# SixLabors/ZlibStream

Measured on AMD Instinct MI355X. Metric: deflate MB/s (input) at level 6, 64 MiB buffers, higher is better.
Workload: dtype u8; 1 GPU; english64: 1 x 67108864-byte pseudo-random-English (Zipf words of alice29.txt) buffer per GPU, level 6, zlib framing, inputs resident in HBM; level=6, buffer_bytes=67108864, buffers_per_gpu=1, compressed_bytes=27425826, parallelism=independent buffers, 1 GPU(s), no collective in the data path

## Files before the change

### zlibstream_amd/csrc/zs_core.h

```cpp
#pragma once
#include <stdint.h>
#include <vector>

#if defined(__HIPCC__)
#include <hip/hip_runtime.h>
#define ZS_HD __host__ __device__ __forceinline__
#define ZS_HD_NOINLINE __host__ __device__
#else
#define ZS_HD inline
#define ZS_HD_NOINLINE
#endif

namespace zs {

constexpr int kMinMatch = 3;
constexpr int kMaxMatch = 258;
constexpr int kMinLookahead = kMaxMatch + kMinMatch + 1;
constexpr int kWSize = 32768;
constexpr int kWMask = kWSize - 1;
constexpr int kWindowSize = 2 * kWSize;
constexpr int kMaxDist = kWSize - kMinLookahead;
constexpr int kSlideAt = kWindowSize - kMinLookahead;
constexpr int kHashBits = 15;
constexpr int kHashSize = 1 << kHashBits;
// ... 417 lines not shown
        uint32_t cK = acc.mK(p), cK4 = acc.mK4(p);
        if (p == 0) cK = cK4 = kNoMatch;
        Step st = lazy_step(kind, p, pend, cK, cK4, lv);
        if (st.emit) {
            uint32_t sym = st.emit == 1 ? (uint32_t)acc.byte(p - 1) : (((uint32_t)st.dist << 16) | (uint32_t)(st.len - 3));
            sink(ns, sym, st.emit == 1 ? p : p - 1 + st.len, p);
            ns++;
        }
        if (st.kind == kXK) pend = cK;
        else if (st.kind == kXK4) pend = cK4;
        kind = st.kind;
        p = st.pos;
    }
    exit_slot = kind == kR ? (int)(p - cx.ce) : 256 + kind;
    nsyms = ns;
}

constexpr int kJumpRounds = 12;
ZS_HD uint32_t node_pack(int succ, int cnt) { return (uint32_t)succ | ((uint32_t)cnt << 14); }
ZS_HD int node_succ(uint32_t v) { return (int)(v & 0x3FFF); }
ZS_HD int node_cnt(uint32_t v) { return (int)(v >> 14); }
ZS_HD uint32_t node_jump(uint32_t v, uint32_t w) { return node_pack(node_succ(w), node_cnt(v) + node_cnt(w)); }

constexpr int kNodeExit3 = 3 * kChunk;
static_assert(kNodeExit3 + 512 <= (1 << 14), "node ids and exit codes share 14 bits");
ZS_HD int kind_row(int kind) { return kind == kR ? 0 : kind == kXK4 ? 2 : 1; }
ZS_HD int node_of3(int kind, int64_t p, int64_t cs, int64_t ce) {
    return p < ce ? kind_row(kind) * kChunk + (int)(p - cs) : kNodeExit3 + (kind == kR ? (int)(p - ce) : 256 + kind);
}
template <class Acc>
ZS_HD uint32_t node_step3(const Acc &acc, int row, int64_t p, int64_t cs, int64_t ce, const LevelCfg &lv) {
    const uint32_t before = acc.mK(p - 1);
    const int kind = row == 0 ? kR : row == 2 ? kXK4 : (before != kNoMatch ? kXK : kL);
    const uint32_t pend = kind == kXK ? before : kind == kXK4 ? acc.mK4(p - 1) : kNoMatch;
    uint32_t cK = acc.mK(p), cK4 = acc.mK4(p);
    if (p == 0) cK = cK4 = kNoMatch;
    const Step st = lazy_step(kind, p, pend, cK, cK4, lv);
    return node_pack(node_of3(st.kind, st.pos, cs, ce), st.emit ? 1 : 0);
}
template <class Acc>
ZS_HD void node_step3_all(const Acc &acc, int64_t p, int64_t cs, int64_t ce, const LevelCfg &lv, uint32_t &r0, uint32_t &r1, uint32_t &r2) {
    const uint32_t before = acc.mK(p - 1), before4 = acc.mK4(p - 1);
    uint32_t cK = acc.mK(p), cK4 = acc.mK4(p);
    if (p == 0) cK = cK4 = kNoMatch;
    const Step s0 = lazy_step(kR, p, kNoMatch, cK, cK4, lv);
    const Step s1 = lazy_step(before != kNoMatch ? kXK : kL, p, before, cK, cK4, lv);
    const Step s2 = lazy_step(kXK4, p, before4, cK, cK4, lv);
    r0 = node_pack(node_of3(s0.kind, s0.pos, cs, ce), s0.emit ? 1 : 0);
    r1 = node_pack(node_of3(s1.kind, s1.pos, cs, ce), s1.emit ? 1 : 0);
    r2 = node_pack(node_of3(s2.kind, s2.pos, cs, ce), s2.emit ? 1 : 0);
}
template <class Acc, class Tbl>
ZS_HD uint32_t chunk_exit_by_table3(const Acc &acc, const Tbl &tbl, const ChunkCtx &cx, int slot, const LevelCfg &lv, int strategy) {
    const int64_t ce = cx.ce;
    int kind, ns;
    int64_t p;
    uint32_t flags;
    NullSink nsink;
    NullEv nev;
    chunk_special_prefix(acc, nsink, cx, slot, lv, strategy, kind, p, ns, flags, nev);
    while (p < ce && (kind == kL || kind == kXK) && ((kind == kXK) != (acc.mK(p - 1) != kNoMatch))) {
        const uint32_t pend = kind == kXK ? acc.mK(p - 1) : kNoMatch;
        uint32_t cK = acc.mK(p), cK4 = acc.mK4(p);
        if (p == 0) cK = cK4 = kNoMatch;
        const Step st = lazy_step(kind, p, pend, cK, cK4, lv);
        if (st.emit) ns++;
        kind = st.kind;
        p = st.pos;
    }
    int node = node_of3(kind, p, cx.cs, ce);
    while (node < kNodeExit3) {
        const uint32_t v = tbl[node];
        ns += node_cnt(v);
        node = node_succ(v);
    }
    return (uint32_t)(node - kNodeExit3) | flags | ((uint32_t)ns << 16);
}

constexpr int kSpecSlabPad = 32;
constexpr int kSpecMaxLenBits = 11;
ZS_HD constexpr int spec_slab_stride(int len_bits) { return (1 << len_bits) + kSpecSlabPad; }
ZS_HD int sym_len(uint32_t sym) { return (sym >> 16) ? (int)(sym & 0xFFFFu) + kMinMatch : 1; }
ZS_HD int spec_cut_index(uint32_t base, int count) {
    const uint32_t i = (base / (uint32_t)kBlockSyms + 1u) * (uint32_t)kBlockSyms - 1u - base;
    return i < (uint32_t)count ? (int)i : -1;
}
ZS_HD int64_t spec_first_start(int64_t cs, int slot) { return slot <= 256 ? cs + slot : cs - 1; }
ZS_HD int64_t spec_sym_end(int64_t start, uint32_t sym) { return start + sym_len(sym); }
ZS_HD int64_t spec_sym_top(int64_t start, bool odd) { return start + (odd ? 2 : 1); }
struct SpecSlabSink {
    uint32_t *out;
    int odd;
    ZS_HD void operator()(int i, uint32_t sym, int64_t end, int64_t top) {
        out[i] = sym;
        if (top != spec_sym_top(end - sym_len(sym), false)) odd = i;
    }
};

ZS_HD bool slot_valid(const ChunkCtx &cx, int slot, int64_t body_end) {
    if (slot <= 256) return cx.cs + slot <= body_end + 257;
    return cx.cs > 0;
}


ZS_HD int extra_lbits(int code) { return code < 8 ? 0 : (code == 28 ? 0 : (code - 4) >> 2); }
ZS_HD int extra_dbits(int code) { return code < 4 ? 0 : (code - 2) >> 1; }
ZS_HD int extra_blbits(int code) { return code == 16 ? 2 : code == 17 ? 3 : code == 18 ? 7 : 0; }
ZS_HD int base_length(int code) {
    if (code < 8) return code;
    if (code == 28) return 0;
    int e = (code - 4) >> 2;
    return ((4 + (code & 3)) << e);
}
ZS_HD int length_code(int lc) {
    if (lc < 8) return lc;
    if (lc == 255) return 28;
    int e = 31 - __builtin_clz((unsigned)lc) - 2;
    return 4 * e + 4 + ((lc >> e) & 3);
}
ZS_HD int base_dist(int code) {
    if (code < 4) return code;
    int e = (code - 2) >> 1;
    return (2 + (code & 1)) << e;
}
ZS_HD int dist_code(int d) {
    if (d < 4) return d;
    int e = 31 - __builtin_clz((unsigned)d) - 1;
    return 2 * e + 2 + ((d >> e) & 1);
}
ZS_HD int bl_order(int i) {
    const uint8_t t[19] = {16, 17, 18, 0, 8, 7, 9, 6, 10, 5, 11, 4, 12, 3, 13, 2, 14, 1, 15};
    return t[i];
}
ZS_HD unsigned bit_reverse(unsigned code, int len) {
    unsigned r = 0;
    for (int i = 0; i < len; i++) {
        r = (r << 1) | (code & 1u);
        code >>= 1;
    }
    return r;
}
ZS_HD int static_llen(int n) { return n <= 143 ? 8 : n <= 255 ? 9 : n <= 279 ? 7 : 8; }
ZS_HD unsigned static_lcode(int n) {
    unsigned c = n <= 143 ? 0x30 + n : n <= 255 ? 0x190 + (n - 144) : n <= 279 ? (unsigned)(n - 256) : 0xC0 + (n - 280);
    return bit_reverse(c, static_llen(n));
}

struct CtData {
    uint16_t fc;
    uint16_t dl;
};

struct TreeWork {
    CtData ltree[kHeapSize];
    CtData dtree[2 * kDCodes + 1];
    CtData bltree[2 * kBlCodes + 1];
    uint16_t heap[kHeapSize];
    uint8_t depth[kHeapSize];
    uint16_t bl_count[kMaxBits + 1];
    int heap_len, heap_max;
    int opt_len, static_len;
    int l_max_code, d_max_code, max_blindex;
};

struct TreeDesc {
    int which;
    int elems, max_length, extra_base;
};
ZS_HD int desc_extra(const TreeDesc &d, int n) {
    if (n < d.extra_base) return 0;
    n -= d.extra_base;
    return d.which == 0 ? extra_lbits(n) : d.which == 1 ? extra_dbits(n) : extra_blbits(n);
}
ZS_HD int desc_static_len(const TreeDesc &d, int n) { return d.which == 0 ? static_llen(n) : 5; }

ZS_HD_NOINLINE inline void gen_bitlen(TreeWork &w, CtData *tree, int max_code, const TreeDesc &d) {
    int h, n, m, bits, overflow = 0;
    for (bits = 0; bits <= kMaxBits; bits++) w.bl_count[bits] = 0;
    tree[w.heap[w.heap_max]].dl = 0;
    for (h = w.heap_max + 1; h < kHeapSize; h++) {
        n = w.heap[h];
        bits = tree[tree[n].dl].dl + 1;
        if (bits > d.max_length) {
            bits = d.max_length;
            overflow++;
        }
        tree[n].dl = (uint16_t)bits;
        if (n > max_code) continue;
        w.bl_count[bits]++;
        int xbits = desc_extra(d, n);
        int f = tree[n].fc;
        w.opt_len += f * (bits + xbits);
        if (d.which != 2) w.static_len += f * (desc_static_len(d, n) + xbits);
    }
    if (overflow == 0) return;
    do {
        bits = d.max_length - 1;
        while (w.bl_count[bits] == 0) bits--;
        w.bl_count[bits]--;
        w.bl_count[bits + 1] += 2;
        w.bl_count[d.max_length]--;
        overflow -= 2;
    } while (overflow > 0);
    for (bits = d.max_length; bits != 0; bits--) {
        n = w.bl_count[bits];
        while (n != 0) {
            m = w.heap[--h];
            if (m > max_code) continue;
            if (tree[m].dl != (unsigned)bits) {
                w.opt_len += bits * (int)tree[m].fc;
                w.opt_len -= (int)tree[m].dl * (int)tree[m].fc;
                tree[m].dl = (uint16_t)bits;
            }
            n--;
        }
    }
}

ZS_HD_NOINLINE inline void gen_codes(CtData *tree, int max_code, const uint16_t *bl_count) {
    uint16_t next_code[kMaxBits + 1];
    unsigned code = 0;
    next_code[0] = 0;
    for (int bits = 1; bits <= kMaxBits; bits++) {
        code = (code + bl_count[bits - 1]) << 1;
        next_code[bits] = (uint16_t)code;
    }
    for (int n = 0; n <= max_code; n++) {
        int len = tree[n].dl;
        if (len == 0) continue;
        tree[n].fc = (uint16_t)bit_reverse(next_code[len]++, len);
    }
}

ZS_HD uint32_t hk_pack(uint32_t freq, uint32_t depth, uint32_t node) { return (freq << 16) | (depth << 10) | node; }
ZS_HD void pqdownheap_packed(uint32_t *hk, int len, int k) {
    const uint32_t v = hk[k];
    int j = k << 1;
    while (j <= len) {
        uint32_t c = hk[j];
        const uint32_t c1 = hk[j + 1];
        const int gj = j << 1;
        const uint32_t g0 = hk[gj], g1 = hk[gj + 1], g2 = hk[gj + 2], g3 = hk[gj + 3];
        if (j < len && (c1 >> 10) <= (c >> 10)) c = c1, j++;
        if ((v >> 10) <= (c >> 10)) break;
        hk[k] = c;
        k = j;
        j <<= 1;
        if (j > len) break;
        uint32_t e = (k & 1) ? g2 : g0;
        const uint32_t e1 = (k & 1) ? g3 : g1;
        if (j < len && (e1 >> 10) <= (e >> 10)) e = e1, j++;
        if ((v >> 10) <= (e >> 10)) break;
        hk[k] = e;
        k = j;
        j <<= 1;
    }
    hk[k] = v;
}
ZS_HD_NOINLINE inline int build_tree(TreeWork &w, uint32_t *hk, CtData *tree, const TreeDesc &d) {
    int max_code = -1, node, len = 0;
    w.heap_max = kHeapSize;
    for (int n = 0; n < d.elems; n++) {
        if (tree[n].fc != 0) {
            hk[++len] = hk_pack(tree[n].fc, 0, (uint32_t)(max_code = n));
        } else {
            tree[n].dl = 0;
        }
    }
    while (len < 2) {
        node = max_code < 2 ? ++max_code : 0;
        hk[++len] = hk_pack(1, 0, (uint32_t)node);
        tree[node].fc = 1;
        w.opt_len--;
        if (d.which != 2) w.static_len -= desc_static_len(d, node);
    }
    for (int n = len / 2; n >= 1; n--) pqdownheap_packed(hk, len, n);
    node = d.elems;
    do {
        const uint32_t n = hk[1];
        hk[1] = hk[len--];
        pqdownheap_packed(hk, len, 1);
        const uint32_t m = hk[1];
        w.heap[--w.heap_max] = (uint16_t)(n & 1023u);
        w.heap[--w.heap_max] = (uint16_t)(m & 1023u);
        const uint32_t f = (n >> 16) + (m >> 16), dn = (n >> 10) & 63u, dm = (m >> 10) & 63u;
        tree[node].fc = (uint16_t)f;
        tree[n & 1023u].dl = tree[m & 1023u].dl = (uint16_t)node;
        hk[1] = hk_pack(f, (dn >= dm ? dn : dm) + 1, (uint32_t)node);
        node++;
        pqdownheap_packed(hk, len, 1);
    } while (len >= 2);
    w.heap[--w.heap_max] = (uint16_t)(hk[1] & 1023u);
    w.heap_len = len;
    gen_bitlen(w, tree, max_code, d);
    gen_codes(tree, max_code, w.bl_count);
    return max_code;
}

ZS_HD_NOINLINE inline void scan_tree(TreeWork &w, CtData *tree, int max_code) {
    int prevlen = -1, curlen, nextlen = tree[0].dl, count = 0, max_count = 7, min_count = 4;
    if (nextlen == 0) max_count = 138, min_count = 3;
    tree[max_code + 1].dl = 0xFFFF;
    for (int n = 0; n <= max_code; n++) {
        curlen = nextlen;
        nextlen = tree[n + 1].dl;
        if (++count < max_count && curlen == nextlen) continue;
        if (count < min_count) {
            w.bltree[curlen].fc += (uint16_t)count;
        } else if (curlen != 0) {
            if (curlen != prevlen) w.bltree[curlen].fc++;
            w.bltree[16].fc++;
        } else if (count <= 10) {
            w.bltree[17].fc++;
        } else {
            w.bltree[18].fc++;
        }
        count = 0;
        prevlen = curlen;
        if (nextlen == 0) max_count = 138, min_count = 3;
        else if (curlen == nextlen) max_count = 6, min_count = 3;
        else max_count = 7, min_count = 4;
    }
}

ZS_HD_NOINLINE inline int build_block_trees(TreeWork &w, uint32_t *hk, int stored_len, bool can_store, int strategy) {
    w.opt_len = w.static_len = 0;
    for (int i = 0; i < kBlCodes; i++) w.bltree[i].fc = 0;
    const TreeDesc ld = {0, kLCodes, kMaxBits, kLiterals + 1};
    const TreeDesc dd = {1, kDCodes, kMaxBits, 0};
    const TreeDesc bd = {2, kBlCodes, kMaxBlBits, 0};
    w.l_max_code = build_tree(w, hk, w.ltree, ld);
    w.d_max_code = build_tree(w, hk, w.dtree, dd);
    scan_tree(w, w.ltree, w.l_max_code);
    scan_tree(w, w.dtree, w.d_max_code);
    build_tree(w, hk, w.bltree, bd);
    int mb;
    for (mb = kBlCodes - 1; mb >= 3; mb--)
        if (w.bltree[bl_order(mb)].dl != 0) break;
    w.max_blindex = mb;
    w.opt_len += 3 * (mb + 1) + 5 + 5 + 4;
    int opt_lenb = (w.opt_len + 3 + 7) >> 3;
    int static_lenb = (w.static_len + 3 + 7) >> 3;
    if (static_lenb <= opt_lenb) opt_lenb = static_lenb;
    if (stored_len + 4 <= opt_lenb && can_store) return 0;
    if (strategy == kFixed || static_lenb == opt_lenb) return 1;
    return 2;
}

template <class LT, class DT>
ZS_HD int encode_symbol(const LT &lt, const DT &dt, int dist, int lc, uint64_t &bits) {
    if (dist == 0) {
        bits = lt[lc].fc;
        return lt[lc].dl;
    }
    int code = length_code(lc);
    uint64_t b = lt[code + kLiterals + 1].fc;
    int n = lt[code + kLiterals + 1].dl;
    int extra = extra_lbits(code);
    if (extra) {
        b |= (uint64_t)(lc - base_length(code)) << n;
        n += extra;
    }
    int d = dist - 1;
    code = dist_code(d);
    b |= (uint64_t)dt[code].fc << n;
    n += dt[code].dl;
    extra = extra_dbits(code);
    if (extra) {
        b |= (uint64_t)(d - base_dist(code)) << n;
        n += extra;
    }
    bits = b;
    return n;
}

struct StaticLTree {
    struct E {
        uint16_t fc, dl;
    };
    ZS_HD E operator[](int n) const { return {(uint16_t)static_lcode(n), (uint16_t)static_llen(n)}; }
};
struct StaticDTree {
    struct E {
        uint16_t fc, dl;
    };
    ZS_HD E operator[](int n) const { return {(uint16_t)bit_reverse((unsigned)n, 5), 5}; }
};


template <class Put>
ZS_HD_NOINLINE inline void emit_tree_rle(const CtData *tree, int max_code, const CtData *bl, Put &put) {
    int prevlen = -1, curlen, nextlen = tree[0].dl, count = 0, max_count = 7, min_count = 4;
    if (nextlen == 0) max_count = 138, min_count = 3;
    for (int n = 0; n <= max_code; n++) {
        curlen = nextlen;
        nextlen = tree[n + 1].dl;
        if (++count < max_count && curlen == nextlen) continue;
        if (count < min_count) {
            do put(bl[curlen].fc, bl[curlen].dl);
            while (--count != 0);
        } else if (curlen != 0) {
            if (curlen != prevlen) {
                put(bl[curlen].fc, bl[curlen].dl);
                count--;
            }
            put(bl[16].fc, bl[16].dl);
            put((unsigned)(count - 3), 2);
        } else if (count <= 10) {
            put(bl[17].fc, bl[17].dl);
            put((unsigned)(count - 3), 3);
        } else {
            put(bl[18].fc, bl[18].dl);
            put((unsigned)(count - 11), 7);
        }
        count = 0;
        prevlen = curlen;
        if (nextlen == 0) max_count = 138, min_count = 3;
        else if (curlen == nextlen) max_count = 6, min_count = 3;
        else max_count = 7, min_count = 4;
    }
}

template <class Put>
ZS_HD_NOINLINE inline void emit_dyn_header(const TreeWork &w, Put &put) {
    int lcodes = w.l_max_code + 1, dcodes = w.d_max_code + 1, blcodes = w.max_blindex + 1;
    put((unsigned)(lcodes - 257), 5);
    put((unsigned)(dcodes - 1), 5);
    put((unsigned)(blcodes - 4), 4);
    for (int rank = 0; rank < blcodes; rank++) put(w.bltree[bl_order(rank)].dl, 3);
    emit_tree_rle(w.ltree, lcodes - 1, w.bltree, put);
    emit_tree_rle(w.dtree, dcodes - 1, w.bltree, put);
}

ZS_HD unsigned zlib_header(int level) {
    unsigned header = (8u + (7u << 4)) << 8;
    unsigned lf = (((unsigned)(level - 1)) & 0xFF) >> 1;
    if (lf > 3) lf = 3;
    header |= lf << 6;
    header += 31 - (header % 31);
    return header;
}

constexpr uint32_t kAdlerBase = 65521;
ZS_HD uint32_t adler_combine(uint32_t a1, uint32_t a2, uint64_t len2) {
    uint32_t rem = (uint32_t)(len2 % kAdlerBase);
    uint32_t s1a = a1 & 0xFFFF, s2a = a1 >> 16, s1b = a2 & 0xFFFF, s2b = a2 >> 16;
    uint64_t s1 = (uint64_t)s1a + s1b + kAdlerBase - 1;
    uint64_t s2 = (uint64_t)s2a + s2b + (uint64_t)rem * ((s1a + kAdlerBase - 1) % kAdlerBase);
    return (uint32_t)(((s2 % kAdlerBase) << 16) | (s1 % kAdlerBase));
}

struct FlushAcct {
// ... 167 lines not shown
```

### zlibstream_amd/csrc/zs_engine.hip

```cpp
#include <hip/hip_runtime.h>

#include <algorithm>
#include <cstdio>
#include <cstdlib>
#include <cstring>
#include <string>
#include <thread>
#include <vector>

#define ZS_BUILDING_LIBRARY
#include "../../include/zsgpu.h"
#include "zs_kernels.hip"
#include "zs_inflate_par.hip"
#include "zs_inflate_tok.hip"
#include "zs_png.hip"
#include "zs_crc32.hip"

using namespace zs;

namespace {

struct DevBuf {
    void *p = nullptr;
    size_t cap = 0;
};

enum Stage {
    kStClear, kStAdler, kStLinks, kStMatch, kStChunkMap, kStSegMap, kStResolve, kStExpand, kStEmitSyms, kStTail, kStTrees,
    kStOffsets, kStEmitBits, kStSpecWalk, kStSpecVerify, kStCrc32, kStSpecCompact, kStPngExpand, kStCount
};
const char *const kStageNames[kStCount] = {"clear", "adler", "links", "match", "chunkmap", "segmap", "resolve", "expand",
                                           "emit_syms", "tail", "trees", "offsets", "emit_bits", "spec_walk", "spec_verify", "crc32_frame",
                                           "spec_compact", "png_expand"};

}

struct zs_ctx {
    int device = 0;
    hipStream_t stream = nullptr;
    hipStream_t aux = nullptr;
    hipEvent_t ev_fork = nullptr, ev_join = nullptr, ev_pre0 = nullptr, ev_pre = nullptr;
    hipEvent_t ev_spec[4] = {};
    std::string err;
    bool profiling = false;
    int fast_fallbacks = 0;
    int round_runs = 0;
    int cut_rounds = 0;
    int lit_fallbacks = 0;
    int spec_streams = 0, spec_fallbacks = 0, spec_wrong_chunks = 0;
    int spec_periodic = 0;
    int64_t dbg_blk_off = 0, dbg_chunk_off = 0, dbg_nchunks = 0, dbg_spec_n = 0, dbg_n_spec = 0;
    int64_t lit_engine_bytes = 0;
    std::vector<int64_t> inf_used;
    int64_t *inf_probe = nullptr;
    int inf_lane_streams = 0;
    int inf_wave_streams = 0;
    int64_t png_segments = 0;
    int fast_rounds = 0;
    bool no_rounds_once = false;
    int last_op = 0;
    hipEvent_t ev[kStCount + 1] = {};
    double stage_ms[kStCount] = {};
    uint32_t *crc_tab = nullptr;
    DevBuf sd, st, work, wpre, geo, link, mm, maps, chunk_far, segmap, supmap, seg_entry, seg_symbase, seg_stale, entry, symbase, stale, syms, blk_end, blk_top, blocks, trees, info, pieces, scratch,
        stage_in, stage_out, wr, inf_desc, inf_state, par_ps, par_st, par_work, par_cbits, par_ccnt, par_surv, par_scnt, par_cands, par_tabs, par_toktabs, par_toks, par_ctoks, par_tokstat, par_tails, par_retry, par_fxtab, par_blocks, par_cells,
        par_windows, par_fail, run_syms, run_bits, run_scratch, run_outs, run_fail, adl_tr, adl_res, plan_blk, ins_bits, mm_bak, cut_pos, cut_bkt, win_groups, win_sg, win_maps, win_entries, persist_bak, resume_flag, rle_tiles, own_in, fr_chunks, fr_meta, fr_planes, fr_prov, fr_base, fr_counters, spec_rec, spec_flags, spec_syms, png_img, png_seg, png_ctr, png_fimg, png_scratch, png_a7img, png_inflated, png_passes, crc_desc, crc_res, png_zs, png_gather, png_ximg, png_raw;
    uint32_t *crc32_tab = nullptr;
    hipEvent_t ev_crc[2] = {};
    hipEvent_t ev_expand[2] = {};
    bool resume_poisoned = false;
    void *pinned = nullptr;
    size_t pinned_cap = 0;
    void *pin_io = nullptr;
    size_t pin_io_cap = 0;
    bool pin_io_busy = false;
    void *pin_out = nullptr;
    size_t pin_out_cap = 0;
    bool pin_out_busy = false;
};

namespace {

bool fail(zs_ctx *c, const char *what, hipError_t e) {
    c->err = std::string(what) + ": " + hipGetErrorString(e);
    return false;
}
#define ZS_HIP(c, call)                                  \
    do {                                                 \
        hipError_t e_ = (call);                          \
        if (e_ != hipSuccess) return fail(c, #call, e_); \
    } while (0)

bool ensure(zs_ctx *c, DevBuf &b, size_t bytes) {
    if (bytes <= b.cap) return true;
    if (b.p) (void)hipFree(b.p);
    b.p = nullptr;
    b.cap = 0;
    size_t want = bytes + bytes / 8 + 4096;
    if (hipMalloc(&b.p, want) != hipSuccess) {
        (void)hipGetLastError();
        b.p = nullptr;
        want = bytes + 4096;
        if (hipMalloc(&b.p, want) != hipSuccess) {
            (void)hipGetLastError();
            b.p = nullptr;
            char msg[160];
            snprintf(msg, sizeof msg, "workspace: %zu bytes do not fit the device's free memory (the pipeline needs ~17 bytes per input byte: split the batch)", bytes);
            c->err = msg;
            return false;
        }
    }
    b.cap = want;
    return true;
}
bool ensure_pinned(zs_ctx *c, size_t bytes) {
    if (bytes <= c->pinned_cap) return true;
    if (c->pinned) (void)hipHostFree(c->pinned);
    c->pinned = nullptr;
    c->pinned_cap = 0;
    ZS_HIP(c, hipHostMalloc(&c->pinned, bytes + 4096, hipHostMallocDefault));
    c->pinned_cap = bytes + 4096;
    return true;
}

struct WorkList {
    std::vector<int32_t> pre;
    void add(int stream, int64_t count) {
        while ((int)pre.size() <= stream) pre.push_back(pre.empty() ? 0 : pre.back());
        pre.push_back(pre.back() + (int32_t)count);
    }
    void finish(int n) {
        if (pre.empty()) pre.push_back(0);
        while ((int)pre.size() <= n) pre.push_back(pre.back());
    }
    size_t size() const { return pre.empty() ? 0 : (size_t)pre.back(); }
    bool empty() const { return size() == 0; }
};
constexpr int kWorkLists = 9;
struct Plan {
    std::vector<StreamDesc> sd;
    WorkList w_clear, w_adler, w_links, w_match, w_chunks, w_segs, w_sups, w_blocks, w_runs;
    int64_t n_pos = 0, n_syms = 0;
    int64_t n_chunks = 0, n_segs = 0, n_sups = 0, n_blocks = 0, n_pieces = 0, n_runs = 0;
    int64_t n_spec = 0;
    int max_spec_n = 0, n_spec_streams = 0;
    bool any_fv = false, any_rle = false;
    bool any_dual = false;
    int64_t n_rle_tiles = 0;
    int64_t lit_bytes = 0;
    std::vector<FsChunk> fr_chunks;
    size_t fr_prov = 0;
    int fr_max_n = 0;
    int64_t n_cuts = 0;
    std::vector<int32_t> seg_c0, seg_after, seg_base, seg_S, seg_cl, cstart, head;
    std::vector<uint32_t> cl;
    std::vector<BlockRec> plan_blk;
    std::vector<int32_t> plan_wr_blk;
};

template <class T>
T *dev(DevBuf &b) {
    return (T *)b.p;
}

struct WriteSpec {
    std::vector<int64_t> ends;
    std::vector<uint8_t> flush;
    int chunk = 512;
    bool raw = false;
    bool flushing() const {
        for (uint8_t f : flush)
            if (f) return true;
        return false;
    }
};

struct RunOpts {
    bool final_run = true, cont = false;
    int64_t hist = 0;
    LitPersist *persist = nullptr;
    int64_t abs_off = 0;
    uint32_t adler_stream = 1, carry_byte = 0;
    int64_t end_bits = 0;
    int64_t stop_abs = -1;
    bool resume = false, mid_write = false, at_read = false;
    int64_t p0 = 0, E0 = 0, base0 = 0, start_block = 0;
    int slot = 0;
    uint32_t start_syms = 0;
};

bool run_pipeline(zs_ctx *c, int n, const void *const *in, const int64_t *in_len, void *const *out, const int64_t *out_cap,
                  int64_t *out_len, int *status, int level, int strategy, int hash_variant, hipStream_t stream,
                  const WriteSpec *const *writes = nullptr, int force_seq = 0, RunOpts *ro = nullptr, bool rounds = false,
                  const std::vector<uint8_t> *force_lit = nullptr) {
    if (level == -1) level = 6;
    LevelCfg lv = level_cfg(level);
    static const bool host_times = getenv("ZS_HOST_TIMES") != nullptr;
    const auto ht0 = std::chrono::steady_clock::now();
    auto ht_us = [&]() { return std::chrono::duration<double, std::micro>(std::chrono::steady_clock::now() - ht0).count(); };
    double ht_plan = 0, ht_launched = 0;
    for (int i = 0; i < n; i++) {
        out_len[i] = 0;
        if (status) status[i] = ZS_STREAM_ERROR;
    }
    bool any_writes = false;
    for (int i = 0; i < n && writes; i++) any_writes = any_writes || writes[i] != nullptr;
    if (any_writes && n > 1)
        for (int i = 0; i < n; i++)
            if (ro || (writes[i] && writes[i]->flushing())) {
                c->err = "flush modes and incremental runs take one stream a call";
                return false;
            }
    std::vector<WriteSpec> rle_one;
    std::vector<const WriteSpec *> rle_writes;
    if (any_writes && strategy == kRle && level >= 1 && !ro && !getenv("ZS_NO_RLE_MULTI")) {
        rle_one.resize((size_t)n);
        rle_writes.assign(writes, writes + n);
// ... 141 lines not shown
                    pl.seg_S.push_back(0), pl.seg_cl.push_back((int32_t)pl.cl.size());
                    s.nsegs++;
                }
            pl.seg_cl.push_back((int32_t)pl.cl.size());
            pl.cstart.push_back(0);
        }
        s.seg_c0 = s.seg_after = s.seg_base = s.seg_S = s.seg_cl = nullptr, s.cl = nullptr, s.cstart = nullptr, s.head = nullptr;
        pl.n_segs += s.nsegs;
        s.sup_off = (int32_t)pl.n_sups;
        pl.n_sups += (s.nsegs + kSupSegs - 1) / kSupSegs;
        s.spec = 0, s.spec_n = 0, s.spec_off = (int32_t)pl.n_spec;
        bool spec_geo = s.body_end >= 0 && geo.body_end == len - kMinLookahead;
        if (spec_geo) {
            const int64_t want = 1 + (len > kWindowSize ? (len - kWindowSize - 1) / kWSize + 1 : 0);
            spec_geo = (int64_t)geo.nsegs() == want && geo.seg_cl.size() == (size_t)want + 1 && geo.seg_cl[0] == 0 && geo.seg_cl[1] == 0;
            for (int64_t k = 1; k < want && spec_geo; k++)
                spec_geo = geo.seg_cl[(size_t)k + 1] - geo.seg_cl[(size_t)k] == 1 &&
                           geo.cl[(size_t)geo.seg_cl[(size_t)k]] == ((uint32_t)(kWindowSize + kWSize * (k - 1)) | kClWindowBit);
        }
        if (spec_on && lv.func == 2 && (strategy == kDefault || strategy == kFiltered) && !wr && !ro && !lit_forced && spec_geo && len >= spec_min &&
            n <= 65535) {
            s.spec = 1, s.spec_n = (int32_t)((((int64_t)s.body_end + kMinLookahead - 1) >> spec_bits) + 1);
            pl.n_spec += s.spec_n, pl.n_spec_streams++;
            pl.max_spec_n = std::max(pl.max_spec_n, (int)s.spec_n);
        }
        s.run_chunk = run_chunk;
        s.fast_runs = fast_par ? (force_seq == 2 ? 1 : (int32_t)((len + run_chunk - 1) / run_chunk)) : 0;
        s.run_slots = fast_par ? (force_seq == 2 ? (int32_t)((len + 4096) / kFastChunk + 1) : s.fast_runs) : 0;
        s.run_off = (int32_t)pl.n_runs;
        pl.n_runs += s.run_slots;
        pl.w_runs.add(i, s.fast_runs);
        s.blk_off = (int32_t)pl.n_blocks;
        s.max_blocks = (int32_t)(level == 0 ? len / 8191 + len / 32506 + 4 : len / kBlockSyms + 2);
        if (flushing) s.max_blocks += (int32_t)wr->ends.size() + 1;
        s.plan_blk = nullptr, s.plan_nblk = 0;
        s.final_run = final_run ? 1 : 0, s.cont = cont ? 1 : 0, s.persist = ro ? ro->persist : nullptr;
        s.abs_off = (ro && !resume) ? ro->abs_off : 0, s.adler_stream = ro ? ro->adler_stream : 1, s.carry_byte = ro ? ro->carry_byte : 0;
        if (level == 0 && strategy != kRle && !ro) {
            const size_t first = pl.plan_blk.size();
            const std::vector<int64_t> no_ends;
            const std::vector<uint8_t> no_flush;
            if (flushing) pl.plan_wr_blk.assign(wr->ends.size(), 0);
            plan_stored_blocks(len, (multi || flushing) ? wr->ends : no_ends, flushing ? wr->flush : no_flush,
                               [&](int64_t start, int32_t blen, int can_store, int eof) {
                                   pl.plan_blk.push_back(BlockRec{start, 0, blen, 0, can_store, eof});
                               },
                               [&](int w, int nb) {
                                   if (flushing) pl.plan_wr_blk[(size_t)w] = nb;
                               });
            s.plan_nblk = (int32_t)(pl.plan_blk.size() - first);
            s.plan_blk = (const BlockRec *)(uintptr_t)first;
            s.max_blocks = s.plan_nblk + 1;
        }
        pl.n_blocks += s.max_blocks;
        s.adler_off = (int32_t)pl.n_pieces;
        s.n_adler = ro ? 0 : (int32_t)((len + kAdlerPiece - 1) / kAdlerPiece);
        pl.n_pieces += s.n_adler;
        pl.w_clear.add(i, (s.out_cap + 65535) / 65536);
        pl.w_adler.add(i, s.n_adler);
        if (s.body_end >= 0 || s.fast_runs > 0 || s.fv_end >= 0)
            pl.w_links.add(i, len - 5 > 0 ? (len - 5 + link_span - 1) / link_span : 0);
        if (s.body_end >= 0) {
            pl.w_match.add(i, (int64_t)s.body_end / kMatchTile + 1);
            pl.w_chunks.add(i, s.nchunks);
            pl.w_segs.add(i, s.nsegs);
            if (s.nsegs > kSupSegs) pl.w_sups.add(i, (s.nsegs + kSupSegs - 1) / kSupSegs);
        }
        pl.w_blocks.add(i, s.max_blocks);
        if (s.body_end < 0 && s.fv_end < 0 && s.rle_end < 0 && s.fast_runs == 0 && s.plan_nblk == 0 && !(level == 0 && strategy != kRle && !ro)) {
            const int64_t from = resume ? ro->p0 : ro ? ro->hist : 0;
            pl.lit_bytes += std::max<int64_t>(0, len - from - (kMinLookahead - 1));
        }
    }
    {
        int64_t need = 0;
        for (int i = 0; i < n; i++) need += (pl.sd[(size_t)i].spec_n + 63) / 64;
        if (pl.n_spec && (int64_t)((pl.max_spec_n + 63) / 64) * n > 4 * need + 4096) {
            for (int i = 0; i < n; i++) pl.sd[(size_t)i].spec = 0, pl.sd[(size_t)i].spec_n = 0, pl.sd[(size_t)i].spec_off = 0;
            pl.n_spec = 0, pl.max_spec_n = 0, pl.n_spec_streams = 0;
        }
    }
    if (allow_dual && dual_broken) {
        allow_dual = false, dual_broken = false;
        goto plan_again;
    }
    pl.any_dual = allow_dual;
    c->lit_engine_bytes += pl.lit_bytes;
    auto plan_rerun = [&]() { c->lit_engine_bytes -= pl.lit_bytes; };
    c->fast_rounds = 0;
    const bool no_rounds_this_call = c->no_rounds_once;
    c->no_rounds_once = false;
    if (pl.any_fv && !getenv("ZS_FAST_NO_ROUNDS") && !no_rounds_this_call && !(ro && ro->resume && getenv("ZS_NO_RESUME_ROUNDS"))) {
        int64_t pos_fv = 0, max_fv = 0;
        for (int i = 0; i < n; i++)
            if (pl.sd[(size_t)i].fv_end >= 0) {
                pos_fv += pl.sd[(size_t)i].fv_end + 1 - pl.sd[(size_t)i].start_pos;
                max_fv = std::max<int64_t>(max_fv, pl.sd[(size_t)i].fv_end + 1 - pl.sd[(size_t)i].start_pos);
            }
        const double t_stream = (double)max_fv / (level >= 3 ? 20e6 : level == 2 ? 35e6 : 46e6);
        const double t_rounds = std::min(0.016, (double)max_fv / 60e6) + (double)pos_fv / 3.5e9;
        if (getenv("ZS_FR_RATIO") ? (double)pos_fv <= atof(getenv("ZS_FR_RATIO")) * (double)max_fv : t_rounds < t_stream) {
            int64_t target = getenv("ZS_FR_CHUNK") ? atoll(getenv("ZS_FR_CHUNK")) : pos_fv / 250;
            target = target < 2048 ? 2048 : target > kFsChunkMax ? kFsChunkMax : target;
            bool too_short = false;
            for (;;) {
                pl.fr_chunks.clear();
                pl.fr_max_n = 0;
                too_short = false;
                for (int i = 0; i < n; i++) {
                    StreamDesc &s = pl.sd[(size_t)i];
                    if (s.fv_end < 0) continue;
                    s.fr_first = (int32_t)pl.fr_chunks.size();
                    {
                        const int32_t *after = pl.seg_after.data() + s.seg_off;
                        const bool res = s.resume != 0;
                        const int64_t shortest = fs_build_chunks(i, (int64_t)s.fv_end, s.nsegs - 1, [&](int k) { return (int64_t)after[k - 1] - (kMinLookahead - 1); }, (int)target, pl.fr_chunks,
                                                                 res ? 2 : 1, res ? s.start_pos : 0);
                        if (shortest < kFsMinSpan) too_short = true;
                    }
                    s.fr_n = (int32_t)pl.fr_chunks.size() - s.fr_first;
                    pl.fr_max_n = s.fr_n > pl.fr_max_n ? s.fr_n : pl.fr_max_n;
                }
                if (pl.fr_chunks.size() <= 256 || target >= kFsChunkMax || getenv("ZS_FR_CHUNK")) break;
                target += 128;
            }
            if (too_short) {
                pl.fr_chunks.clear();
                pl.fr_max_n = 0;
                for (int i = 0; i < n; i++) pl.sd[(size_t)i].fr_first = pl.sd[(size_t)i].fr_n = 0;
            }
            for (FsChunk &ck : pl.fr_chunks) {
                ck.prov_off = (uint32_t)pl.fr_prov;
                pl.fr_prov += (size_t)(ck.b_hi - ck.b_lo) + kMaxMatch + 64;
            }
            if (pl.fr_prov > 0xFFFF0000u) {
                pl.fr_chunks.clear();
                pl.fr_max_n = 0, pl.fr_prov = 0;
                for (int i = 0; i < n; i++) pl.sd[(size_t)i].fr_first = pl.sd[(size_t)i].fr_n = 0;
            }
        }
    }
    WorkList *const lists[kWorkLists] = {&pl.w_clear, &pl.w_adler, &pl.w_links, &pl.w_match, &pl.w_chunks, &pl.w_segs, &pl.w_sups, &pl.w_blocks, &pl.w_runs};
    for (WorkList *l : lists) l->finish(n);
    size_t n_work = pl.w_clear.size() + pl.w_adler.size() + pl.w_links.size() + pl.w_match.size() + pl.w_chunks.size() +
                    pl.w_segs.size() + pl.w_sups.size() + pl.w_blocks.size() + pl.w_runs.size();
    if (!ensure(c, c->sd, sizeof(StreamDesc) * (size_t)n) || !ensure(c, c->st, sizeof(StreamState) * (size_t)n) ||
        !ensure(c, c->work, sizeof(uint2) * (n_work + 1)) || !ensure(c, c->link, 2 * (size_t)pl.n_pos + 64) ||
        !ensure(c, c->mm, 8 * (size_t)pl.n_pos + 256) ||
        !ensure(c, c->maps, 4 * (size_t)(pl.n_chunks + 1) * kSlots) || !ensure(c, c->segmap, 8 * (size_t)(pl.n_segs + 1) * kSlots) ||
        !ensure(c, c->supmap, 8 * (size_t)(pl.n_sups + 1) * kSlots) || !ensure(c, c->chunk_far, 2 * (size_t)pl.n_chunks + 64) ||
        !ensure(c, c->seg_entry, 2 * (size_t)(pl.n_segs + 2)) || !ensure(c, c->seg_symbase, 4 * (size_t)(pl.n_segs + 2)) ||
        !ensure(c, c->seg_stale, (size_t)pl.n_segs + 64) || !ensure(c, c->entry, 2 * (size_t)(pl.n_chunks + 2)) ||
        !ensure(c, c->symbase, 4 * (size_t)(pl.n_chunks + 2)) || !ensure(c, c->stale, (size_t)pl.n_chunks + 64) ||
        !ensure(c, c->syms, 4 * (size_t)pl.n_syms + 64) || !ensure(c, c->blk_end, 4 * (size_t)pl.n_blocks + 64) ||
        !ensure(c, c->blk_top, 4 * (size_t)pl.n_blocks + 64) || !ensure(c, c->blocks, sizeof(BlockRec) * (size_t)pl.n_blocks) ||
        !ensure(c, c->trees, sizeof(TreeWork) * (size_t)pl.n_blocks) || !ensure(c, c->info, sizeof(BlockInfo) * (size_t)pl.n_blocks) ||
        !ensure(c, c->pieces, 4 * (size_t)pl.n_pieces + 64) || !ensure(c, c->scratch, (size_t)kScratchBytes * (size_t)n) ||
        !ensure(c, c->cut_pos, 8 * (size_t)pl.n_cuts + 64) || !ensure(c, c->cut_bkt, 8 * (size_t)pl.n_cuts + 64) ||
        (pl.n_spec && (!ensure(c, c->spec_rec, 8 * (size_t)pl.n_spec + 64) || !ensure(c, c->spec_flags, 4 * (size_t)n + 64) ||
                       !ensure(c, c->spec_syms, 4 * (size_t)pl.n_spec * (size_t)spec_slab_stride(spec_bits) + 64))))
        return false;
    const size_t o_segcl = 16 * (size_t)pl.n_segs, o_cstart = o_segcl + 4 * ((size_t)pl.n_segs + (size_t)n),
                 o_head = o_cstart + 4 * ((size_t)pl.n_chunks + (size_t)n), o_cl = o_head + 4 * (size_t)pl.n_chunks;
    const size_t geo_bytes = o_cl + 4 * pl.cl.size();
    if (!ensure(c, c->geo, geo_bytes + 64)) return false;
    for (int i = 0; i < n; i++) {
        StreamDesc &s = pl.sd[(size_t)i];
        const int32_t *g = (const int32_t *)c->geo.p;
        const uint8_t *gb = (const uint8_t *)c->geo.p;
        s.seg_c0 = g + s.seg_off, s.seg_after = g + pl.n_segs + s.seg_off, s.seg_base = g + 2 * pl.n_segs + s.seg_off;
        s.seg_S = g + 3 * pl.n_segs + s.seg_off;
        s.seg_cl = (const int32_t *)(gb + o_segcl) + s.seg_off + i;
        s.cstart = (const int32_t *)(gb + o_cstart) + s.chunk_off + i;
        s.head = (const int32_t *)(gb + o_head) + s.chunk_off;
        s.cl = (const uint32_t *)(gb + o_cl);
    }
    if (pl.any_fv) {
        if (!ensure(c, c->ins_bits, (size_t)pl.n_pos / 8 + kFvBitSlack)) return false;
        for (int i = 0; i < n; i++)
            if (pl.sd[(size_t)i].fv_end >= 0) pl.sd[(size_t)i].ins_bits = dev<uint32_t>(c->ins_bits) + pl.sd[(size_t)i].pos_off / 32;
    }
    if (!pl.plan_blk.empty()) {
        if (!ensure(c, c->plan_blk, sizeof(BlockRec) * pl.plan_blk.size())) return false;
        for (int i = 0; i < n; i++)
            if (pl.sd[(size_t)i].plan_nblk) pl.sd[(size_t)i].plan_blk = dev<BlockRec>(c->plan_blk) + (uintptr_t)pl.sd[(size_t)i].plan_blk;
    }
    if (pl.n_runs &&
        (!ensure(c, c->run_syms, 4 * (size_t)pl.n_runs * kFastRunSyms) || !ensure(c, c->run_bits, 4 * (size_t)pl.n_runs * kFastRunBitWords) ||
         !ensure(c, c->run_scratch, (size_t)pl.n_runs * kFastRunScratch) || !ensure(c, c->run_outs, sizeof(FastRunOut) * (size_t)pl.n_runs) ||
         !ensure(c, c->run_fail, 4 * (size_t)n + 64)))
        return false;
    if (any_writes) {
        std::vector<size_t> nws((size_t)n, 0), offs;
        for (int i = 0; i < n; i++) {
            const WriteSpec *wr = writes[i];
            if (wr && (wr->ends.size() > 1 || wr->flushing() || ro)) nws[(size_t)i] = wr->ends.size();
        }
        const size_t wr_bytes = layout_write_blocks(nws, offs);
        if (!ensure(c, c->wr, wr_bytes + 64)) return false;
        std::vector<uint8_t> hw(rounds ? 0 : wr_bytes + 64, 0);
        for (int i = 0; i < n; i++) {
            const WriteSpec *wr = writes[i];
            const size_t nw = nws[(size_t)i];
            if (!wr || !(wr->ends.size() > 1 || wr->flushing() || ro)) continue;
            uint8_t *blk = (uint8_t *)c->wr.p + offs[(size_t)i];
            pl.sd[(size_t)i].wr_end = (const int64_t *)blk;
            if (wr->flushing() || ro) {
                pl.sd[(size_t)i].wr_blk = (int32_t *)(blk + 8 * nw);
                pl.sd[(size_t)i].wr_flush = blk + 12 * nw;
            }
            if (rounds || !nw) continue;
            memcpy(hw.data() + offs[(size_t)i], wr->ends.data(), sizeof(int64_t) * nw);
            if (wr->flushing() || ro) memcpy(hw.data() + offs[(size_t)i] + 12 * nw, wr->flush.data(), nw);
            if (!pl.plan_wr_blk.empty()) memcpy(hw.data() + offs[(size_t)i] + 8 * nw, pl.plan_wr_blk.data(), 4 * nw);
        }
        if (!rounds && wr_bytes) {
            ZS_HIP(c, hipMemcpyAsync(c->wr.p, hw.data(), hw.size(), hipMemcpyHostToDevice, stream));
            ZS_HIP(c, hipStreamSynchronize(stream));
        }
    }
    if (!rounds && !pl.plan_blk.empty()) {
        ZS_HIP(c, hipMemcpyAsync(c->plan_blk.p, pl.plan_blk.data(), sizeof(BlockRec) * pl.plan_blk.size(), hipMemcpyHostToDevice, stream));
        ZS_HIP(c, hipStreamSynchronize(stream));
    }
    const size_t pre_bytes = 4 * (size_t)kWorkLists * (size_t)(n + 1);
    size_t up_bytes = sizeof(StreamDesc) * (size_t)n + pre_bytes + geo_bytes + 16;
    if (!ensure_pinned(c, std::max(up_bytes, sizeof(StreamState) * (size_t)n)) || !ensure(c, c->wpre, pre_bytes + 64)) return false;
    uint8_t *hp = (uint8_t *)c->pinned;
    memcpy(hp, pl.sd.data(), sizeof(StreamDesc) * (size_t)n);
    int32_t *hpre = (int32_t *)(hp + sizeof(StreamDesc) * (size_t)n);
    size_t o_clear = 0, o_adler, o_links, o_match, o_chunks, o_segs, o_sups, o_blocks, o_runs;
    WorkOffsets wo;
    {
        size_t *const offs[kWorkLists] = {&o_clear, &o_adler, &o_links, &o_match, &o_chunks, &o_segs, &o_sups, &o_blocks, &o_runs};
        size_t at = 0;
        for (int l = 0; l < kWorkLists; l++) {
            *offs[l] = at;
            wo.off[l] = (uint32_t)at;
            memcpy(hpre + (size_t)l * (size_t)(n + 1), lists[l]->pre.data(), 4 * (size_t)(n + 1));
            at += lists[l]->size();
        }
        wo.off[kWorkLists] = (uint32_t)at;
    }
    if (geo_bytes) {
        uint8_t *hg = hp + sizeof(StreamDesc) * (size_t)n + pre_bytes;
        if (pl.n_segs) {
            memcpy(hg, pl.seg_c0.data(), 4 * (size_t)pl.n_segs);
            memcpy(hg + 4 * (size_t)pl.n_segs, pl.seg_after.data(), 4 * (size_t)pl.n_segs);
            memcpy(hg + 8 * (size_t)pl.n_segs, pl.seg_base.data(), 4 * (size_t)pl.n_segs);
            memcpy(hg + 12 * (size_t)pl.n_segs, pl.seg_S.data(), 4 * (size_t)pl.n_segs);
        }
        memcpy(hg + o_segcl, pl.seg_cl.data(), 4 * pl.seg_cl.size());
        memcpy(hg + o_cstart, pl.cstart.data(), 4 * pl.cstart.size());
        if (pl.n_chunks) memcpy(hg + o_head, pl.head.data(), 4 * (size_t)pl.n_chunks);
        if (!pl.cl.empty()) memcpy(hg + o_cl, pl.cl.data(), 4 * pl.cl.size());
        if (!rounds) ZS_HIP(c, hipMemcpyAsync(c->geo.p, hg, geo_bytes, hipMemcpyHostToDevice, stream));
    }
    if (!rounds) ZS_HIP(c, hipMemcpyAsync(c->sd.p, hp, sizeof(StreamDesc) * (size_t)n, hipMemcpyHostToDevice, stream));
    if (n_work && !rounds) {
        ZS_HIP(c, hipMemcpyAsync(c->wpre.p, hpre, pre_bytes, hipMemcpyHostToDevice, stream));
        hipLaunchKernelGGL(zs_worklist_kernel, dim3((unsigned)((n_work + 255) / 256)), dim3(256), 0, stream, dev<int32_t>(c->wpre), n, wo,
                           dev<uint2>(c->work));
    }
    if (!rounds) {
        ZeroRegions z;
        auto reg = [&](int r, DevBuf &b, size_t bytes) {
            z.p[r] = b.p;
            z.n16[r] = (uint32_t)(((bytes + 15) / 16 < b.cap / 16) ? (bytes + 15) / 16 : b.cap / 16);
        };
        reg(0, c->stale, (size_t)pl.n_chunks + 64);
        reg(1, c->seg_stale, (size_t)pl.n_segs + 64);
        reg(2, c->st, sizeof(StreamState) * (size_t)n);
        if (pl.any_fv) reg(3, c->ins_bits, (size_t)pl.n_pos / 8 + kFvBitSlack);
        else z.p[3] = nullptr, z.n16[3] = 0;
        uint32_t most = 0;
        for (int r = 0; r < 4; r++) most = z.n16[r] > most ? z.n16[r] : most;
        unsigned blocks = (most + 255) / 256;
        if (blocks > 2048) blocks = 2048;
        if (blocks < 1) blocks = 1;
        hipLaunchKernelGGL(zs_zero_kernel, dim3(blocks), dim3(256), 0, stream, z);
        if (ro && ro->resume && pl.sd[0].fv_end >= 0) {
            const int64_t lo = std::max<int64_t>(0, ro->p0 - kWSize - 64) / 32, hi = ro->p0 / 32;
            if (hi > lo) ZS_HIP(c, hipMemsetAsync(pl.sd[0].ins_bits + lo, 0xFF, (size_t)(hi - lo) * 4, stream));
            ZS_HIP(c, hipMemsetD32Async((hipDeviceptr_t)(pl.sd[0].ins_bits + hi), (int)((1u << (ro->p0 & 31)) - 1u), 1, stream));
        }
    }

    const StreamDesc *d_sd = dev<StreamDesc>(c->sd);
    StreamState *d_st = dev<StreamState>(c->st);
    const uint2 *d_work = dev<uint2>(c->work);
    const bool prof = c->profiling;
    const int k5_ahead = getenv("ZS_K5_AHEAD") ? atoi(getenv("ZS_K5_AHEAD")) : 1;
    c->dbg_blk_off = pl.sd[0].blk_off, c->dbg_chunk_off = pl.sd[0].chunk_off, c->dbg_nchunks = pl.sd[0].nchunks;
    c->dbg_spec_n = pl.sd[0].spec_n, c->dbg_n_spec = pl.n_spec;
    const K5Spec k5s{dev<uint32_t>(c->spec_rec), dev<uint32_t>(c->spec_rec) + pl.n_spec, spec_bits, spec_warm, spec_corrupt,
                     dev<uint32_t>(c->spec_syms), spec_slab_stride(spec_bits)};
    int spec_ok_streams = 0;
    bool need_maps = true, spec_ran = false;
    if (!rounds) c->spec_streams = c->spec_fallbacks = c->spec_wrong_chunks = c->spec_periodic = 0;
    auto mark = [&](int i) {
        if (prof) (void)hipEventRecord(c->ev[i], stream);
    };
    ht_plan = ht_us();
    ZS_HIP(c, hipEventRecord(c->ev_pre0, stream));
    auto side_work = [&]() -> bool {
        ZS_HIP(c, hipStreamWaitEvent(c->aux, c->ev_pre0, 0));
        if (!pl.w_clear.empty())
            hipLaunchKernelGGL(zs_clear_kernel, dim3((unsigned)pl.w_clear.size()), dim3(256), 0, c->aux, d_sd, d_work + o_clear);
        if (!pl.w_adler.empty())
// ... 210 lines not shown
                    char b[64];
                    snprintf(b, sizeof b, " %u/%d(%.2f)", changed, fr.range, r <= g_n ? 0.0 : std::chrono::duration<double, std::milli>(t_now - t_last).count());
                    t_last = t_now;
                    trace += b;
                }
                if (!env_fixed) {
                    static const double env_wake = getenv("ZS_FR_WAKE") ? atof(getenv("ZS_FR_WAKE")) : 4.0;
                    const size_t awake = std::min<size_t>(nch, (size_t)(env_wake * (double)changed));
                    const int tail = env_tail;
                    fr.range = std::min<int>(range_max, std::max<int>(tail, (int)((awake + 255) / 256)));
                }
            }
            c->fast_rounds = r;
            if (env_dbg) fprintf(stderr, "zs: DeflateFast over %zu chunks of %d streams, up to %d to a workgroup: %d rounds (changed/range:%s)\n", nch, n, range_max, r, trace.c_str());
            if (changed) {
                ZS_HIP(c, hipStreamSynchronize(c->aux));
                c->no_rounds_once = true;
                return plan_rerun(), run_pipeline(c, n, in, in_len, out, out_cap, out_len, status, level, strategy, hash_variant, stream, writes, force_seq, ro, false, force_lit);
            }
            const FsMeta *mf = dev<FsMeta>(c->fr_meta) + (size_t)((r - 1) & 1) * nch;
            hipLaunchKernelGGL(zs_fast_commit_scan_kernel, dim3((unsigned)n), dim3(1024), 0, stream, d_sd, d_st, mf, dev<int32_t>(c->fr_base));
            hipLaunchKernelGGL(zs_fast_commit_kernel, dim3((unsigned)nch), dim3(256), 0, stream, d_sd, fr, mf, dev<int32_t>(c->fr_base), dev<uint16_t>(c->link),
                               dev<uint32_t>(c->syms), dev<int32_t>(c->blk_end), dev<int32_t>(c->blk_top));
        } else {
            hipLaunchKernelGGL((zs_fast_sweep_kernel<1024, kFsTile1, false>), dim3((unsigned)n), dim3(1024), fs_lds, stream, d_sd, d_st, dev<uint16_t>(c->link),
                               dev<uint32_t>(c->syms), dev<int32_t>(c->blk_end), dev<int32_t>(c->blk_top), lv, strategy, FsRounds());
        }
    }
    if (pl.any_rle) {
        const size_t nt = (size_t)pl.n_rle_tiles;
        if (!ensure(c, c->rle_tiles, 4 * (4 * nt + (size_t)n) + 256)) return false;
        int32_t *rb = dev<int32_t>(c->rle_tiles);
        RleTiles rt{rb, rb + nt, rb + 2 * nt, rb + 3 * nt, rb + 4 * nt};
        int max_tiles = 0;
        for (int i = 0; i < n; i++)
            if (pl.sd[(size_t)i].rle_end >= 0) max_tiles = std::max(max_tiles, (pl.sd[(size_t)i].rle_end + kMaxMatch + 1 + 4095) / 4096);
        auto tiles = [&](auto &&launch) {
            for (int s0 = 0; s0 < n; s0 += 65535) launch(dim3((unsigned)((max_tiles + 3) / 4), (unsigned)std::min(n - s0, 65535)), s0);
        };
        tiles([&](dim3 tg, int s0) { hipLaunchKernelGGL(zs_rle_starts_kernel, tg, dim3(256), 0, stream, d_sd, rt, s0); });
        hipLaunchKernelGGL(zs_rle_scan_kernel, dim3((unsigned)n), dim3(1024), 0, stream, d_sd, rt);
        tiles([&](dim3 tg, int s0) {
            hipLaunchKernelGGL(zs_rle_pass_kernel<0>, tg, dim3(256), 0, stream, d_sd, rt, dev<uint32_t>(c->syms), dev<int32_t>(c->blk_end), dev<int32_t>(c->blk_top), s0);
        });
        hipLaunchKernelGGL(zs_rle_sums_kernel, dim3((unsigned)n), dim3(1024), 0, stream, d_sd, d_st, rt);
        tiles([&](dim3 tg, int s0) {
            hipLaunchKernelGGL(zs_rle_pass_kernel<1>, tg, dim3(256), 0, stream, d_sd, rt, dev<uint32_t>(c->syms), dev<int32_t>(c->blk_end), dev<int32_t>(c->blk_top), s0);
        });
    }
    const bool tail_late = ro && (!ro->final_run || ro->resume);
    const bool tail_serial = !tail_late && n >= 64 && (pl.n_pos / n >= (96 << 10) || getenv("ZS_TAIL_SERIAL")) && !getenv("ZS_TAIL_FORK");
    if (!tail_late && !tail_serial) {
        ZS_HIP(c, hipEventRecord(c->ev_fork, stream));
        ZS_HIP(c, hipStreamWaitEvent(c->aux, c->ev_fork, 0));
        hipLaunchKernelGGL(zs_tail_kernel, dim3((unsigned)n), dim3(1024), kTailLds, c->aux, d_sd, d_st, dev<uint16_t>(c->link),
                           dev<uint32_t>(c->syms), dev<int32_t>(c->blk_end), dev<int32_t>(c->blk_top), dev<BlockRec>(c->blocks),
                           dev<uint8_t>(c->scratch), c->crc_tab, lv, strategy, hash_variant, level);
        ZS_HIP(c, hipEventRecord(c->ev_join, c->aux));
    }
    if (!pl.w_segs.empty() && need_maps)
        hipLaunchKernelGGL(zs_expand_kernel, dim3((unsigned)((pl.w_segs.size() + 63) / 64)), dim3(64), 0, stream, d_sd, d_st,
                           d_work + o_segs, (int)pl.w_segs.size(), dev<uint2>(c->mm), dev<uint16_t>(c->link),
                           dev<uint32_t>(c->maps), dev<uint16_t>(c->seg_entry), dev<uint32_t>(c->seg_symbase),
                           dev<uint8_t>(c->stale), dev<uint16_t>(c->entry), dev<uint32_t>(c->symbase), c->crc_tab, lv, strategy,
                           hash_variant);
    mark(8);
    if (!pl.w_chunks.empty() && need_maps)
        hipLaunchKernelGGL((zs_emit_syms_lane_kernel<4, 0>), dim3((unsigned)((pl.w_chunks.size() + 63) / 64)), dim3(kK5Threads), 0, stream, d_sd, d_st,
                           d_work + o_chunks, (int)pl.w_chunks.size(), dev<uint2>(c->mm), dev<uint16_t>(c->link), dev<uint16_t>(c->entry),
                           dev<uint32_t>(c->symbase), dev<uint32_t>(c->syms), dev<int32_t>(c->blk_end), dev<int32_t>(c->blk_top),
                           c->crc_tab, lv, strategy, hash_variant, k5_ahead, k5s);
    if (spec_ok_streams) {
        if (prof) (void)hipEventRecord(c->ev_spec[2], stream);
        hipLaunchKernelGGL(zs_spec_compact_kernel, dim3((unsigned)((pl.max_spec_n + 3) / 4), (unsigned)n), dim3(256), 0, stream, d_sd, d_st, k5s,
                           dev<uint32_t>(c->syms), dev<int32_t>(c->blk_end), dev<int32_t>(c->blk_top));
        if (prof) (void)hipEventRecord(c->ev_spec[3], stream);
    }
    mark(9);
    if (tail_serial)
        hipLaunchKernelGGL(zs_tail_kernel, dim3((unsigned)n), dim3(1024), kTailLds, stream, d_sd, d_st, dev<uint16_t>(c->link),
                           dev<uint32_t>(c->syms), dev<int32_t>(c->blk_end), dev<int32_t>(c->blk_top), dev<BlockRec>(c->blocks),
                           dev<uint8_t>(c->scratch), c->crc_tab, lv, strategy, hash_variant, level);
    else if (!tail_late) ZS_HIP(c, hipStreamWaitEvent(stream, c->ev_join, 0));
    hipLaunchKernelGGL(zs_body_blocks_kernel, dim3((unsigned)n), dim3(256), 0, stream, d_sd, d_st, dev<int32_t>(c->blk_end),
                       dev<int32_t>(c->blk_top), dev<BlockRec>(c->blocks), dev<uint32_t>(c->syms));
    if (tail_late)
        hipLaunchKernelGGL(zs_tail_kernel, dim3((unsigned)n), dim3(1024), kTailLds, stream, d_sd, d_st, dev<uint16_t>(c->link),
                           dev<uint32_t>(c->syms), dev<int32_t>(c->blk_end), dev<int32_t>(c->blk_top), dev<BlockRec>(c->blocks),
                           dev<uint8_t>(c->scratch), c->crc_tab, lv, strategy, hash_variant, level);
    if (pl.n_runs) {
        if (!getenv("ZS_FAST_NO_PROBE") && force_seq == 0 && !pl.any_dual) {
            hipLaunchKernelGGL(zs_fast_probe_kernel, dim3((unsigned)n), dim3(256), 0, stream, d_sd, dev<uint16_t>(c->link), dev<int32_t>(c->run_fail));
            std::vector<int32_t> np((size_t)n, 0);
            ZS_HIP(c, hipMemcpyAsync(np.data(), c->run_fail.p, 4 * (size_t)n, hipMemcpyDeviceToHost, stream));
            ZS_HIP(c, hipStreamSynchronize(stream));
            for (int i = 0; i < n; i++)
                if (np[(size_t)i]) {
                    ZS_HIP(c, hipStreamSynchronize(c->aux));
                    return plan_rerun(), run_pipeline(c, n, in, in_len, out, out_cap, out_len, status, level, strategy, hash_variant, stream, writes, 1, ro, false, force_lit);
                }
        }
        ZS_HIP(c, hipMemsetAsync(c->run_fail.p, 0, 4 * (size_t)n + 64, stream));
        hipLaunchKernelGGL(zs_fast_run_kernel, dim3((unsigned)pl.w_runs.size()), dim3(1024), kFastRunLds, stream, d_sd, d_work + o_runs,
                           dev<uint16_t>(c->link), dev<uint32_t>(c->run_syms), dev<uint32_t>(c->run_bits), dev<uint8_t>(c->run_scratch),
                           dev<FastRunOut>(c->run_outs), c->crc_tab, lv, strategy, hash_variant);
        hipLaunchKernelGGL(zs_fast_verify_kernel, dim3((unsigned)pl.w_runs.size()), dim3(256), 0, stream, d_sd, d_work + o_runs,
                           dev<uint32_t>(c->run_bits), dev<FastRunOut>(c->run_outs), dev<int32_t>(c->run_fail));
        std::vector<int32_t> rfail((size_t)n, 0);
        ZS_HIP(c, hipMemcpyAsync(rfail.data(), c->run_fail.p, 4 * (size_t)n, hipMemcpyDeviceToHost, stream));
        ZS_HIP(c, hipStreamSynchronize(stream));
        for (int i = 0; i < n; i++)
            if (rfail[(size_t)i]) {
                ZS_HIP(c, hipStreamSynchronize(c->aux));
                c->fast_fallbacks++;
                std::vector<FastRunOut> outs((size_t)pl.n_runs);
                ZS_HIP(c, hipMemcpy(outs.data(), c->run_outs.p, sizeof(FastRunOut) * outs.size(), hipMemcpyDeviceToHost));
                if (getenv("ZS_DEBUG"))
                    for (int j = 0; j < pl.sd[(size_t)i].fast_runs; j++) {
                        const FastRunOut &o = outs[(size_t)pl.sd[(size_t)i].run_off + j];
                        fprintf(stderr, "zs: stream %d run %d ok=%d mark=%lld (+%lld syms) end=%lld nsyms=%lld n_ev=%d\n", i, j, o.ok,
                                (long long)o.mark_pos, (long long)o.mark_nsyms, (long long)o.end_pos, (long long)o.nsyms, o.n_ev);
                    }
                double t_engine = 0, t_sweeps = 0;
                for (int k = 0; k < n; k++) {
                    const StreamDesc &sk = pl.sd[(size_t)k];
                    if (sk.fast_runs <= 0) continue;
                    int64_t syms = 0, matches = 0;
                    for (int j = 0; j < sk.fast_runs; j++) syms += outs[(size_t)sk.run_off + j].nsyms, matches += outs[(size_t)sk.run_off + j].n_match;
                    const double scale = sk.fast_runs > 1 ? 0.8 : 1.0;
                    const double te = scale * (1.2e-6 * (double)matches + 0.03e-6 * (double)(syms - matches)) + (double)sk.n / 1.5e9;
                    if (getenv("ZS_DEBUG")) fprintf(stderr, "zs: stream %d: ~%.0f symbols one at a time, ~%.0f in runs of literals, %d bytes\n", k, scale * (double)matches, scale * (double)(syms - matches), sk.n);
                    t_engine = std::max(t_engine, te);
                    t_sweeps = std::max(t_sweeps, (double)sk.n / (level >= 3 ? 20e6 : level == 2 ? 35e6 : 46e6));
                }
                const int mode = (force_seq == 0 && !getenv("ZS_NO_WHOLE_RUNS") && (getenv("ZS_WHOLE_RUNS") || t_engine < 0.7 * t_sweeps)) ? 2 : 1;
                if (getenv("ZS_DEBUG")) fprintf(stderr, "zs: the runs did not verify: %s (engine %.1f ms, sweeps up to %.1f ms)\n", mode == 2 ? "one run per stream" : "the sweeps", t_engine * 1e3, t_sweeps * 1e3);
                return plan_rerun(), run_pipeline(c, n, in, in_len, out, out_cap, out_len, status, level, strategy, hash_variant, stream, writes, mode, ro, false, force_lit);
            }
        hipLaunchKernelGGL(zs_fast_plan_kernel, dim3((unsigned)n), dim3(256), 0, stream, d_sd, d_st, dev<FastRunOut>(c->run_outs), n);
        hipLaunchKernelGGL(zs_fast_stitch_kernel, dim3((unsigned)pl.w_runs.size()), dim3(256), 0, stream, d_sd, d_work + o_runs,
                           dev<uint32_t>(c->run_syms), dev<FastRunOut>(c->run_outs), dev<uint32_t>(c->syms), dev<int32_t>(c->blk_end),
                           dev<int32_t>(c->blk_top));
        hipLaunchKernelGGL(zs_fast_blocks_kernel, dim3((unsigned)n), dim3(64), 0, stream, d_sd, d_st, dev<FastRunOut>(c->run_outs),
                           dev<int32_t>(c->blk_end), dev<int32_t>(c->blk_top), dev<BlockRec>(c->blocks), n);
    }
    mark(10);
    const int trees_threads = pl.w_blocks.size() > 8192 ? 128 : 256;
    if (n >= 64 && !getenv("ZS_NO_LIVE_LIST")) {
        hipLaunchKernelGGL(zs_live_scan_kernel, dim3(1), dim3(1024), 0, stream, d_st, n, dev<int32_t>(c->wpre));
        hipLaunchKernelGGL(zs_live_fill_kernel, dim3((unsigned)((pl.w_blocks.size() + 255) / 256)), dim3(256), 0, stream, dev<int32_t>(c->wpre), n,
                           (uint32_t)pl.w_blocks.size(), dev<uint2>(c->work) + o_blocks);
    }
    hipLaunchKernelGGL(zs_trees_kernel, dim3((unsigned)pl.w_blocks.size()), dim3(trees_threads), 0, stream, d_sd, d_st, d_work + o_blocks,
                       dev<uint32_t>(c->syms), dev<BlockRec>(c->blocks), dev<TreeWork>(c->trees), dev<BlockInfo>(c->info), strategy, level, 2);
    mark(11);
    ZS_HIP(c, hipStreamWaitEvent(stream, c->ev_pre, 0));
    hipLaunchKernelGGL(zs_offsets_kernel, dim3((unsigned)n), dim3(256), 0, stream, d_sd, d_st, dev<BlockRec>(c->blocks),
                       dev<BlockInfo>(c->info), dev<TreeWork>(c->trees), dev<uint32_t>(c->pieces), level, n);
    mark(12);
    hipLaunchKernelGGL(zs_emit_bits_kernel, dim3((unsigned)pl.w_blocks.size()), dim3(256), 0, stream, d_sd, d_st, d_work + o_blocks,
                       dev<uint32_t>(c->syms), dev<BlockRec>(c->blocks), dev<TreeWork>(c->trees), dev<BlockInfo>(c->info));
    mark(13);
    ZS_HIP(c, hipGetLastError());
    StreamState *hst = (StreamState *)c->pinned;
    ZS_HIP(c, hipMemcpyAsync(hst, d_st, sizeof(StreamState) * (size_t)n, hipMemcpyDeviceToHost, stream));
    ht_launched = ht_us();
    ZS_HIP(c, hipStreamSynchronize(stream));
    if (host_times) fprintf(stderr, "zs: host: plan + uploads %.0f us, all launched at %.0f us, device done at %.0f us\n", ht_plan, ht_launched, ht_us());
    c->last_op = lv.func == 1 ? 2 : 0;
    if (getenv("ZS_DEBUG_CHAIN") && n == 1) {
        const int64_t q0 = atoll(getenv("ZS_DEBUG_CHAIN")) - (ro ? ro->abs_off : 0);
        if (q0 > 0 && q0 < in_len[0]) {
            std::vector<uint16_t> lk((size_t)in_len[0]);
            (void)hipMemcpy(lk.data(), dev<uint16_t>(c->link) + pl.sd[0].pos_off, 2 * (size_t)in_len[0], hipMemcpyDeviceToHost);
            fprintf(stderr, "[zs] run of %lld bytes (stream position %lld on), resume %d at %lld: chain of %lld:", (long long)in_len[0], (long long)(ro ? ro->abs_off : 0),
                    pl.sd[0].resume, (long long)pl.sd[0].start_pos, (long long)q0);
            int64_t q = q0;
            int hops = 0;
            const int64_t want = getenv("ZS_DEBUG_CHAIN_WANT") ? atoll(getenv("ZS_DEBUG_CHAIN_WANT")) - (ro ? ro->abs_off : 0) : -1;
            int want_at = -1;
            while (lk[(size_t)q] && hops < 100000) {
                q -= lk[(size_t)q], hops++;
                if (hops <= 12) fprintf(stderr, " %lld", (long long)q);
                if (q == want) want_at = hops;
            }
            fprintf(stderr, " ... %d hops, ends at %lld; position %lld is hop %d\n", hops, (long long)q, (long long)want, want_at);
        }
    }
    if (getenv("ZS_DEBUG_FA") && writes && writes[0] && pl.sd[0].wr_blk) {
        const WriteSpec *wr = writes[0];
        const size_t nw = wr->ends.size();
        std::vector<int32_t> wb(nw);
        (void)hipMemcpy(wb.data(), pl.sd[0].wr_blk, 4 * nw, hipMemcpyDeviceToHost);
        fprintf(stderr, "[zs] run of %lld bytes, %zu Writes, %d blocks, body ends at %d, resume %d; blocks before each Write:", (long long)in_len[0], nw, hst[0].nblocks,
                pl.sd[0].body_end, pl.sd[0].resume);
        for (size_t k = 0; k < nw && k < 24; k++) fprintf(stderr, " %d(end %lld, flush %d)", wb[k], (long long)wr->ends[k], wr->flush.empty() ? 0 : wr->flush[k]);
        fprintf(stderr, "\n");
    }
    if (prof) {
        for (int i = 0; i < kStCount; i++) {
            float ms = 0;
            if (i >= kStLinks && i <= kStEmitBits) (void)hipEventElapsedTime(&ms, c->ev[i], c->ev[i + 1]);
            c->stage_ms[i] = ms;
        }
        if (spec_ran) {
            float a = 0, b = 0, m = 0;
            (void)hipEventElapsedTime(&a, c->ev[kStChunkMap], c->ev_spec[0]);
            (void)hipEventElapsedTime(&b, c->ev_spec[0], c->ev_spec[1]);
            (void)hipEventElapsedTime(&m, c->ev_spec[1], c->ev[kStChunkMap + 1]);
            c->stage_ms[kStSpecWalk] = a, c->stage_ms[kStSpecVerify] = b, c->stage_ms[kStChunkMap] = m;
            float k = 0;
            if (spec_ok_streams) (void)hipEventElapsedTime(&k, c->ev_spec[2], c->ev_spec[3]);
            c->stage_ms[kStSpecCompact] = k;
        }
    }
    {
        bool any_poison = false;
        std::vector<uint8_t> fl(force_lit ? *force_lit : std::vector<uint8_t>((size_t)n, 0));
        for (int i = 0; i < n; i++)
            if (hst[i].poison) any_poison = true, fl[(size_t)i] = 1;
        if (any_poison) {
            ZS_HIP(c, hipStreamSynchronize(c->aux));
            if (ro && ro->resume) {
                c->err = "the resumed run met a read the bulk pipeline leaves to the literal engine";
                c->resume_poisoned = true;
                return false;
            }
            c->lit_fallbacks++;
            return plan_rerun(), run_pipeline(c, n, in, in_len, out, out_cap, out_len, status, level, strategy, hash_variant, stream, writes, force_seq, ro, false, &fl);
        }
    }
    if (!ro && !rounds) {
        bool gave_up = false;
        for (int i = 0; i < n; i++) gave_up = gave_up || hst[i].deferred == 1;
        if (gave_up) {
            ZS_HIP(c, hipStreamSynchronize(c->aux));
            c->round_runs++;
            if (!run_cut_rounds()) return false;
            return plan_rerun(), run_pipeline(c, n, in, in_len, out, out_cap, out_len, status, level, strategy, hash_variant, stream, writes, force_seq, ro, true, force_lit);
        }
    }
    if (ro) ro->end_bits = hst[0].end_bits;
    bool all_ok = true;
    for (int i = 0; i < n; i++) {
        out_len[i] = hst[i].out_len;
        if (status) status[i] = hst[i].status;
        if (hst[i].status != 0 && all_ok) {
            c->err = hst[i].status == ZS_BUF_ERROR ? "buffer error"
                                                   : "stored block larger than the reference's pending buffer (the managed engine throws here)";
            all_ok = false;
        }
    }
    return all_ok;
}

bool device_adlers(zs_ctx *c, int m, const void *const *bufs, const int64_t *lens, const void *const *trailers, uint32_t *adlers,
                   int *ok, hipStream_t stream) {
    if (m <= 0) return true;
    std::vector<StreamDesc> sd((size_t)m);
    std::vector<uint2> work;
    int64_t n_pieces = 0;
    for (int i = 0; i < m; i++) {
        StreamDesc &s = sd[(size_t)i];
        memset(&s, 0, sizeof s);
        s.in = (const uint8_t *)bufs[i];
        s.n = (int32_t)lens[i];
        s.adler_off = (int32_t)n_pieces;
        s.n_adler = (int32_t)((lens[i] + kAdlerPiece - 1) / kAdlerPiece);
        n_pieces += s.n_adler;
        for (int k = 0; k < s.n_adler; k++) work.push_back(make_uint2((unsigned)i, (unsigned)k));
    }
    const size_t b_sd = sizeof(StreamDesc) * (size_t)m, b_work = sizeof(uint2) * work.size(), b_tr = sizeof(void *) * (size_t)m;
    if (!ensure(c, c->sd, b_sd) || !ensure(c, c->work, b_work + 16) || !ensure(c, c->pieces, 4 * (size_t)n_pieces + 64) ||
        !ensure(c, c->adl_tr, b_tr) || !ensure(c, c->adl_res, sizeof(uint2) * (size_t)m) ||
        !ensure_pinned(c, b_sd + b_work + b_tr + sizeof(uint2) * (size_t)m))
        return false;
    uint8_t *hp = (uint8_t *)c->pinned;
    memcpy(hp, sd.data(), b_sd);
    if (b_work) memcpy(hp + b_sd, work.data(), b_work);
    if (trailers) memcpy(hp + b_sd + b_work, trailers, b_tr);
    ZS_HIP(c, hipMemcpyAsync(c->sd.p, hp, b_sd, hipMemcpyHostToDevice, stream));
    if (b_work) ZS_HIP(c, hipMemcpyAsync(c->work.p, hp + b_sd, b_work, hipMemcpyHostToDevice, stream));
    if (trailers) ZS_HIP(c, hipMemcpyAsync(c->adl_tr.p, hp + b_sd + b_work, b_tr, hipMemcpyHostToDevice, stream));
    if (!work.empty())
        hipLaunchKernelGGL(zs_adler_kernel, dim3((unsigned)work.size()), dim3(256), 0, stream, dev<StreamDesc>(c->sd), dev<uint2>(c->work),
                           dev<uint32_t>(c->pieces));
    hipLaunchKernelGGL(zs_adler_finish_kernel, dim3((unsigned)m), dim3(256), 0, stream, dev<StreamDesc>(c->sd), dev<uint32_t>(c->pieces),
                       trailers ? (const uint8_t *const *)c->adl_tr.p : nullptr, dev<uint2>(c->adl_res));
    uint2 *hres = (uint2 *)(hp + b_sd + b_work + b_tr);
    ZS_HIP(c, hipMemcpyAsync(hres, c->adl_res.p, sizeof(uint2) * (size_t)m, hipMemcpyDeviceToHost, stream));
    ZS_HIP(c, hipStreamSynchronize(stream));
    for (int i = 0; i < m; i++) {
        if (adlers) adlers[i] = hres[i].x;
        if (ok) ok[i] = (int)hres[i].y;
    }
    return true;
}

int batch_prefix_that_fits(zs_ctx *c, int n, const int64_t *in_len, const int64_t *out_cap, int lo, int per_byte) {
    size_t free_b = 0, total_b = 0;
    if (hipMemGetInfo(&free_b, &total_b) != hipSuccess) return n;
    const DevBuf *held[] = {&c->link, &c->mm, &c->maps, &c->segmap, &c->supmap, &c->syms, &c->trees, &c->blocks, &c->info, &c->stage_in, &c->stage_out,
                            &c->scratch, &c->ins_bits, &c->mm_bak};
    size_t have = 0;
    for (const DevBuf *b : held) have += b->cap;
    const double budget = 0.55 * ((double)free_b + (double)have);
    double need = 0;
    int hi = lo;
    while (hi < n) {
        const double add = (double)in_len[hi] * per_byte + (per_byte > 19 ? (double)out_cap[hi] : 0.0) + 4.0e6;
        if (hi > lo && need + add > budget) break;
        need += add;
        hi++;
    }
    return hi;
}

bool check_args(zs_ctx *c, int n, const int64_t *in_len, int level, int strategy) {
    if (!c) return false;
    if (n < 0 || level < -1 || level > 9 || strategy < 0 || strategy > 4) {
        c->err = "stream error";
        return false;
    }
    for (int i = 0; i < n; i++)
        if (in_len[i] < 0 || in_len[i] > 0x7FFFFFFF - 1024) {
            c->err = "stream error";
            return false;
        }
    return true;
}

}

extern "C" {

void zs_ctx_destroy(zs_ctx *c);
int zs_ctx_create(int device, zs_ctx **out) {
    if (!out) return ZS_STREAM_ERROR;
    *out = nullptr;
    int count = 0;
    if (hipGetDeviceCount(&count) != hipSuccess || count <= 0 || device < 0 || device >= count) return ZS_STREAM_ERROR;
    if (hipSetDevice(device) != hipSuccess) return ZS_STREAM_ERROR;
    zs_ctx *c = new zs_ctx();
    c->device = device;
    if (hipStreamCreateWithFlags(&c->stream, hipStreamNonBlocking) != hipSuccess) {
        zs_ctx_destroy(c);
        return ZS_MEM_ERROR;
    }
    for (auto &e : c->ev) (void)hipEventCreate(&e);
    for (auto &e : c->ev_spec) (void)hipEventCreate(&e);
    for (auto &e : c->ev_crc) (void)hipEventCreate(&e);
    for (auto &e : c->ev_expand) (void)hipEventCreate(&e);
    {
        int *d_ok = nullptr, ok = 0;
        if (hipMalloc((void **)&d_ok, sizeof(int)) != hipSuccess) {
            zs_ctx_destroy(c);
            return ZS_MEM_ERROR;
        }
        hipLaunchKernelGGL(zs_lds_order_kernel, dim3(1), dim3(64), 0, c->stream, d_ok);
        const bool copied = hipMemcpyAsync(&ok, d_ok, sizeof(int), hipMemcpyDeviceToHost, c->stream) == hipSuccess &&
                            hipStreamSynchronize(c->stream) == hipSuccess;
        (void)hipFree(d_ok);
        if (!copied || !ok) {
            fprintf(stderr, "zsgpu: LDS lane-order self-test failed on device %d; this build cannot run there\n", device);
            zs_ctx_destroy(c);
            return ZS_STREAM_ERROR;
        }
    }
    if (hipStreamCreateWithFlags(&c->aux, hipStreamNonBlocking) != hipSuccess ||
        hipEventCreateWithFlags(&c->ev_fork, hipEventDisableTiming) != hipSuccess ||
        hipEventCreateWithFlags(&c->ev_join, hipEventDisableTiming) != hipSuccess ||
        hipEventCreateWithFlags(&c->ev_pre0, hipEventDisableTiming) != hipSuccess ||
        hipEventCreateWithFlags(&c->ev_pre, hipEventDisableTiming) != hipSuccess) {
        zs_ctx_destroy(c);
        return ZS_MEM_ERROR;
    }
    std::vector<uint32_t> tab(1024);
    for (int t = 0; t < 4; t++)
        for (int i = 0; i < 256; i++) tab[(size_t)t * 256 + i] = crc32c_table_entry(t, (uint32_t)i);
    if (hipMalloc((void **)&c->crc_tab, 4096) != hipSuccess ||
        hipMemcpy(c->crc_tab, tab.data(), 4096, hipMemcpyHostToDevice) != hipSuccess ||
        hipFuncSetAttribute((const void *)zs_match_kernel, hipFuncAttributeMaxDynamicSharedMemorySize, kMatchLds + 16) != hipSuccess ||
        hipFuncSetAttribute((const void *)zs_resolve_kernel, hipFuncAttributeMaxDynamicSharedMemorySize, kResolveLds) != hipSuccess ||
        hipFuncSetAttribute((const void *)zs_links_kernel, hipFuncAttributeMaxDynamicSharedMemorySize, kLkLds) != hipSuccess ||
        hipFuncSetAttribute((const void *)zs_tail_kernel, hipFuncAttributeMaxDynamicSharedMemorySize, kTailLds) != hipSuccess ||
        hipFuncSetAttribute((const void *)zs_fast_run_kernel, hipFuncAttributeMaxDynamicSharedMemorySize, kFastRunLds) != hipSuccess ||
        hipFuncSetAttribute((const void *)zs_fast_sweep_kernel<1024, kFsTile1, false>, hipFuncAttributeMaxDynamicSharedMemorySize, (fs_lds_bytes<1024, kFsTile1>())) != hipSuccess ||
        hipFuncSetAttribute((const void *)zs_fast_sweep_kernel<1024, kFsTile1, true>, hipFuncAttributeMaxDynamicSharedMemorySize, (fs_lds_bytes<1024, kFsTile1>())) != hipSuccess ||
        hipFuncSetAttribute((const void *)zs_inf_window_kernel, hipFuncAttributeMaxDynamicSharedMemorySize, kWinMapLds) != hipSuccess ||
        hipFuncSetAttribute((const void *)zs_inf_chain_par_kernel, hipFuncAttributeMaxDynamicSharedMemorySize, kChainParLds) != hipSuccess ||
        hipFuncSetAttribute((const void *)zs_inf_expand_kernel, hipFuncAttributeMaxDynamicSharedMemorySize, kExpLds) != hipSuccess ||
        hipFuncSetAttribute((const void *)zs_cuts_repair_kernel<256, 1>, hipFuncAttributeMaxDynamicSharedMemorySize, kRepairLds) != hipSuccess ||
        hipFuncSetAttribute((const void *)zs_cuts_repair_kernel<256, 8>, hipFuncAttributeMaxDynamicSharedMemorySize, kRepairLds) != hipSuccess ||
        hipFuncSetAttribute((const void *)zs_cuts_repair_kernel<1024, 32>, hipFuncAttributeMaxDynamicSharedMemorySize, kRepairLds) != hipSuccess ||
        hipFuncSetAttribute((const void *)zs_png_unfilter_kernel, hipFuncAttributeMaxDynamicSharedMemorySize, kPngMaxLds) != hipSuccess ||
        hipFuncSetAttribute((const void *)zs_inflate_kernel, hipFuncAttributeMaxDynamicSharedMemorySize, kInfLds) != hipSuccess) {
        zs_ctx_destroy(c);
        return ZS_MEM_ERROR;
    }
    hipFuncAttributes fa;
    if (hipFuncGetAttributes(&fa, (const void *)zs_match_kernel) != hipSuccess || fa.sharedSizeBytes != 0) {
        fprintf(stderr, "zsgpu: zs_match_kernel has static LDS; its tile addressing assumes none\n");
        zs_ctx_destroy(c);
        return ZS_STREAM_ERROR;
    }
    *out = c;
    return ZS_OK;
}

void zs_ctx_destroy(zs_ctx *c) {
    if (!c) return;
    (void)hipSetDevice(c->device);
    DevBuf *bufs[] = {&c->sd, &c->st, &c->work, &c->wpre, &c->geo, &c->link, &c->mm, &c->maps, &c->chunk_far, &c->segmap, &c->supmap, &c->seg_entry, &c->seg_symbase, &c->seg_stale, &c->entry, &c->symbase, &c->stale, &c->syms,
                      &c->blk_end, &c->blk_top, &c->blocks, &c->trees, &c->info, &c->pieces, &c->scratch, &c->stage_in, &c->stage_out, &c->wr, &c->inf_desc, &c->inf_state, &c->par_ps, &c->par_st, &c->par_work, &c->par_cbits, &c->par_ccnt, &c->par_surv, &c->par_scnt,
                      &c->par_cands, &c->par_tabs, &c->par_toktabs, &c->par_toks, &c->par_ctoks, &c->par_tokstat, &c->par_tails, &c->par_retry, &c->par_fxtab, &c->par_blocks, &c->par_cells, &c->par_windows, &c->par_fail, &c->run_syms, &c->run_bits,
                      &c->run_scratch, &c->run_outs, &c->run_fail, &c->adl_tr, &c->adl_res, &c->plan_blk, &c->ins_bits, &c->mm_bak, &c->cut_pos, &c->cut_bkt, &c->win_groups, &c->win_sg, &c->win_maps, &c->win_entries, &c->persist_bak, &c->resume_flag, &c->rle_tiles, &c->own_in, &c->fr_chunks, &c->fr_meta, &c->fr_planes, &c->fr_prov, &c->fr_base, &c->fr_counters, &c->spec_rec, &c->spec_flags, &c->spec_syms, &c->png_img, &c->png_seg, &c->png_ctr, &c->png_fimg, &c->png_scratch, &c->png_a7img, &c->png_inflated, &c->png_passes, &c->crc_desc, &c->crc_res, &c->png_zs, &c->png_gather, &c->png_ximg, &c->png_raw};
    for (DevBuf *b : bufs)
        if (b->p) (void)hipFree(b->p);
    if (c->crc_tab) (void)hipFree(c->crc_tab);
    if (c->crc32_tab) (void)hipFree(c->crc32_tab);
    for (auto &e : c->ev_crc)
        if (e) (void)hipEventDestroy(e);
    for (auto &e : c->ev_expand)
        if (e) (void)hipEventDestroy(e);
    if (c->pinned) (void)hipHostFree(c->pinned);
    if (c->pin_io) (void)hipHostFree(c->pin_io);
    if (c->pin_out) (void)hipHostFree(c->pin_out);
    for (auto &e : c->ev)
        if (e) (void)hipEventDestroy(e);
    for (auto &e : c->ev_spec)
        if (e) (void)hipEventDestroy(e);
    if (c->ev_fork) (void)hipEventDestroy(c->ev_fork);
    if (c->ev_join) (void)hipEventDestroy(c->ev_join);
    if (c->ev_pre0) (void)hipEventDestroy(c->ev_pre0);
    if (c->ev_pre) (void)hipEventDestroy(c->ev_pre);
    if (c->aux) (void)hipStreamDestroy(c->aux);
    if (c->stream) (void)hipStreamDestroy(c->stream);
    delete c;
}

const char *zs_ctx_last_error(const zs_ctx *c) { return c ? c->err.c_str() : "no context"; }

int64_t zs_deflate_bound(int64_t n) { return n + (n >> 3) + 1024; }

void zs_ctx_set_profiling(zs_ctx *c, int enable) {
    if (c) c->profiling = enable != 0;
}
int zs_ctx_stage_count(const zs_ctx *) { return kStCount; }
int64_t zs_ctx_counter(const zs_ctx *c, const char *name) {
    if (!c || !name) return -1;
    const std::string k(name);
    if (k == "fast_rounds") return c->fast_rounds;
    if (k == "fast_fallbacks") return c->fast_fallbacks;
    if (k == "round_runs") return c->round_runs;
    if (k == "cut_rounds") return c->cut_rounds;
    if (k == "lit_fallbacks") return c->lit_fallbacks;
    if (k == "lit_engine_bytes") return c->lit_engine_bytes;
    if (k == "spec_streams") return c->spec_streams;
    if (k == "spec_fallbacks") return c->spec_fallbacks;
    if (k == "spec_periodic") return c->spec_periodic;
    if (k == "spec_wrong_chunks") return c->spec_wrong_chunks;
    if (k == "inf_lane_streams") return c->inf_lane_streams;
    if (k == "inf_wave_streams") return c->inf_wave_streams;
    if (k == "png_segments") return c->png_segments;
    return -1;
}

int64_t zs_ctx_debug_read(zs_ctx *c, const char *name, void *out, int64_t cap) {
    if (!c || !name || !out || !c->st.p) return -1;
    const std::string k(name);
    (void)hipSetDevice(c->device);
    StreamState ss;
    if (hipMemcpy(&ss, c->st.p, sizeof ss, hipMemcpyDeviceToHost) != hipSuccess) return -1;
    const void *src = nullptr;
    int64_t bytes = 0;
    const int32_t state[6] = {ss.tail_p, ss.tail_kind, (int32_t)ss.tail_pend, ss.k_done, ss.preins, (int32_t)ss.body_syms};
    if (k == "state") {
        if (cap < (int64_t)sizeof state) return -1;
        memcpy(out, state, sizeof state);
        return sizeof state;
    }
    if (k == "blk_end") src = dev<int32_t>(c->blk_end) + c->dbg_blk_off, bytes = 4 * (int64_t)(ss.body_syms / kBlockSyms);
    else if (k == "blk_top") src = dev<int32_t>(c->blk_top) + c->dbg_blk_off, bytes = 4 * (int64_t)(ss.body_syms / kBlockSyms);
    else if (k == "symbase") src = dev<uint32_t>(c->symbase) + c->dbg_chunk_off, bytes = 4 * c->dbg_nchunks;
    else if (k == "spec_base") src = dev<uint32_t>(c->spec_rec) + c->dbg_n_spec, bytes = 4 * c->dbg_spec_n;
    else return -1;
    if (bytes > cap || (bytes > 0 && !src)) return -1;
    if (bytes > 0 && hipMemcpy(out, src, (size_t)bytes, hipMemcpyDeviceToHost) != hipSuccess) return -1;
    return bytes;
}

const char *zs_ctx_stage_name(const zs_ctx *c, int s) {
    static const char *const inf_names[6] = {"inf_find", "inf_measure", "inf_chain", "inf_decode", "inf_windows", "inf_resolve"};
    if (s == kStCrc32 || s == kStSpecCompact || s == kStPngExpand) return kStageNames[s];
    if (c && c->last_op == 1) return s >= 0 && s < 6 ? inf_names[s] : "";
    if (c && c->last_op == 2 && s == kStExpand) return "fast_sweep";
    if (c && c->last_op == 2 && s == kStTail) return "fast_runs+tail";
    return s >= 0 && s < kStCount ? kStageNames[s] : "";
}
double zs_ctx_stage_ms(const zs_ctx *c, int s) { return c && s >= 0 && s < kStCount ? c->stage_ms[s] : 0.0; }

int zs_deflate_batch_device(zs_ctx *c, int n, const void *const *in, const int64_t *in_len, void *const *out,
                            const int64_t *out_cap, int64_t *out_len, int *status, int level, int strategy, int hash_variant,
                            void *hip_stream) {
    if (!check_args(c, n, in_len, level, strategy)) return ZS_STREAM_ERROR;
    if (n == 0) return ZS_OK;
    if (hipSetDevice(c->device) != hipSuccess) return ZS_STREAM_ERROR;
    hipStream_t s = hip_stream ? (hipStream_t)hip_stream : c->stream;
    int rc = ZS_OK;
    for (int lo = 0; lo < n;) {
        const int hi = batch_prefix_that_fits(c, n, in_len, out_cap, lo, 19);
        if (!run_pipeline(c, hi - lo, in + lo, in_len + lo, out + lo, out_cap + lo, out_len + lo, status ? status + lo : nullptr, level, strategy,
                          hash_variant, s) && rc == ZS_OK)
            rc = c->err == "buffer error" ? ZS_BUF_ERROR : ZS_STREAM_ERROR;
        lo = hi;
    }
    return rc;
}

int zs_deflate_writes_batch_device(zs_ctx *c, int n, const void *const *in, const int64_t *in_len, const int64_t *const *write_ends,
                                   const int64_t *n_writes, void *const *out, const int64_t *out_cap, int64_t *out_len, int *status, int level,
                                   int strategy, int hash_variant, void *hip_stream) {
    if (!write_ends) return zs_deflate_batch_device(c, n, in, in_len, out, out_cap, out_len, status, level, strategy, hash_variant, hip_stream);
    if (!check_args(c, n, in_len, level, strategy)) return ZS_STREAM_ERROR;
    if (n == 0) return ZS_OK;
    std::vector<WriteSpec> specs((size_t)n);
    std::vector<const WriteSpec *> ptrs((size_t)n, nullptr);
    for (int i = 0; i < n; i++) {
        if (!write_ends[i] || (n_writes && n_writes[i] <= 0)) continue;
        if (!n_writes || !write_list_ends(write_ends[i], n_writes[i], in_len[i], specs[(size_t)i].ends)) {
            c->err = "stream error";
            return ZS_STREAM_ERROR;
        }
        if (specs[(size_t)i].ends.empty()) continue;
        specs[(size_t)i].flush.assign(specs[(size_t)i].ends.size(), 0);
        ptrs[(size_t)i] = &specs[(size_t)i];
    }
    if (hipSetDevice(c->device) != hipSuccess) return ZS_STREAM_ERROR;
    hipStream_t s = hip_stream ? (hipStream_t)hip_stream : c->stream;
    int rc = ZS_OK;
    for (int lo = 0; lo < n;) {
        const int hi = batch_prefix_that_fits(c, n, in_len, out_cap, lo, 19);
        if (!run_pipeline(c, hi - lo, in + lo, in_len + lo, out + lo, out_cap + lo, out_len + lo, status ? status + lo : nullptr, level, strategy,
                          hash_variant, s, ptrs.data() + lo) && rc == ZS_OK)
            rc = c->err == "buffer error" ? ZS_BUF_ERROR : ZS_STREAM_ERROR;
        lo = hi;
    }
    return rc;
}

int zs_deflate_writes_device(zs_ctx *c, const void *in, int64_t in_len, const int64_t *write_ends, int64_t n_writes, void *out,
                             int64_t out_cap, int64_t *out_len, int level, int strategy, int hash_variant, void *hip_stream) {
    if (!check_args(c, 1, &in_len, level, strategy)) return ZS_STREAM_ERROR;
    if (hipSetDevice(c->device) != hipSuccess) return ZS_STREAM_ERROR;
    WriteSpec ws;
    if (!write_list_ends(write_ends, n_writes, in_len, ws.ends)) {
        c->err = "stream error";
        return ZS_STREAM_ERROR;
    }
    ws.flush.assign(ws.ends.size(), 0);
    const WriteSpec *const one = &ws;
    hipStream_t s = hip_stream ? (hipStream_t)hip_stream : c->stream;
    int st = 0;
    if (!run_pipeline(c, 1, &in, &in_len, &out, &out_cap, out_len, &st, level, strategy, hash_variant, s, ws.ends.size() > 1 ? &one : nullptr))
        return c->err == "buffer error" ? ZS_BUF_ERROR : ZS_STREAM_ERROR;
    return ZS_OK;
}
// ... 1610 lines not shown
```

### zlibstream_amd/csrc/zs_kernels.hip

```cpp
#include <hip/hip_runtime.h>

#include <type_traits>

#include "zs_device.h"
#include "zs_png.h"

namespace zs {

typedef uint32_t __attribute__((aligned(1))) u32u;
typedef uint64_t __attribute__((aligned(1))) u64u;
typedef const __attribute__((address_space(1))) uint8_t *gcbytes;
typedef __attribute__((address_space(1))) uint8_t *gbytes_w;
__device__ __forceinline__ gcbytes as_global(const uint8_t *p) { return (gcbytes)(uintptr_t)p; }
__device__ __forceinline__ gbytes_w as_global(uint8_t *p) { return (gbytes_w)(uintptr_t)p; }
typedef const __attribute__((address_space(1))) uint32_t __attribute__((aligned(1))) *gcu32u;
typedef const __attribute__((address_space(1))) uint64_t __attribute__((aligned(1))) *gcu64u;
__device__ __forceinline__ uint32_t g_u32_bytes(gcbytes p) {
    return (uint32_t)p[0] | ((uint32_t)p[1] << 8) | ((uint32_t)p[2] << 16) | ((uint32_t)p[3] << 24);
}
typedef uint32_t u32x4 __attribute__((ext_vector_type(4)));
typedef const __attribute__((address_space(1))) u32x4 *gcu32x4;
__device__ __forceinline__ uint32_t lds_u32(const uint8_t *base, int idx) {
    const uint32_t *q = (const uint32_t *)(base + (idx & ~3));
    return __builtin_amdgcn_alignbyte(q[1], q[0], (uint32_t)idx & 3u);
// ... 2387 lines not shown
    __shared__ int bad;
    const uint2 w = work[blockIdx.x];
    const StreamDesc s = sd[w.x];
    const int j = (int)w.y;
    if (j == 0) return;
    const int64_t run = (int64_t)s.run_off + j;
    const FastRunOut a = outs[run - 1], b = outs[run];
    if (threadIdx.x == 0) bad = (b.mark_pos < 0 || b.mark_pos != a.end_pos);
    __syncthreads();
    if (!bad) {
        const int64_t xa = (j - 1) * (int64_t)s.run_chunk - kFastWarm < 0 ? 0 : (j - 1) * (int64_t)s.run_chunk - kFastWarm;
        const int64_t xb = (int64_t)j * s.run_chunk - kFastWarm < 0 ? 0 : (int64_t)j * s.run_chunk - kFastWarm;
        const uint32_t *ba = run_bits + (run - 1) * kFastRunBitWords, *bb = run_bits + run * kFastRunBitWords;
        int64_t lo = b.mark_pos - kWSize;
        if (lo < 0) lo = 0;
        int mism = 0;
        for (int64_t p = lo + threadIdx.x; p < b.mark_pos; p += 256) {
            const int64_t ia = p - xa, ib = p - xb;
            const uint32_t va = (ba[ia >> 5] >> (ia & 31)) & 1u;
            const uint32_t vb = ib >= 0 ? (bb[ib >> 5] >> (ib & 31)) & 1u : va;
            const uint32_t want = ib >= 0 ? vb : 1u;
            mism |= (va != want);
#ifdef ZS_FV_PROF
            if (va != want && j == 1) printf("VERIFY run %d: position %lld run before has %u, this run %u (mark %lld)\n", j, (long long)p, va, want, (long long)b.mark_pos);
#endif
        }
        if (mism) bad = 1;
        if (threadIdx.x == 0) {
            for (int u = 0; u < a.n_ev; u++) {
                if (a.ev[u] < lo - 1 || a.ev[u] > b.mark_pos) continue;
                bool found = false;
                for (int v = 0; v < b.n_ev; v++) found |= b.ev[v] == a.ev[u];
                if (!found) bad = 1;
#ifdef ZS_FV_PROF
                if (!found && j == 1) printf("VERIFY run %d: event of the run before at %lld not in this run\n", j, (long long)a.ev[u]);
#endif
            }
            for (int v = 0; v < b.n_ev; v++) {
                if (b.ev[v] < lo - 1 || b.ev[v] > b.mark_pos) continue;
                bool found = false;
                for (int u = 0; u < a.n_ev; u++) found |= a.ev[u] == b.ev[v];
                if (!found) bad = 1;
            }
        }
    }
    __syncthreads();
    if (threadIdx.x == 0 && bad) {
        outs[run].ok = 0;
        stream_fail[w.x] = 1;
    }
}

__global__ __launch_bounds__(256) void zs_fast_plan_kernel(const StreamDesc *sd, StreamState *st, FastRunOut *outs, int nstreams) {
    __shared__ long long part[256];
    __shared__ long long carry;
    const int si = blockIdx.x, tid = threadIdx.x;
    if (si >= nstreams) return;
    const StreamDesc s = sd[si];
    if (s.fast_runs <= 0) return;
    if (tid == 0) carry = 0;
    __syncthreads();
    for (int j0 = 0; j0 < s.fast_runs; j0 += 256) {
        const int j = j0 + tid;
        const long long own = j < s.fast_runs ? (long long)(outs[s.run_off + j].nsyms - outs[s.run_off + j].mark_nsyms) : 0;
        part[tid] = own;
        __syncthreads();
        for (int o = 1; o < 256; o <<= 1) {
            const long long x = tid >= o ? part[tid - o] : 0;
            __syncthreads();
            part[tid] += x;
            __syncthreads();
        }
        if (j < s.fast_runs) outs[s.run_off + j].sym_dst = carry + part[tid] - own;
        __syncthreads();
        if (tid == 255) carry += part[255];
        __syncthreads();
    }
    if (tid == 0) {
        const long long total = carry;
        st[si].nsyms = (uint32_t)total;
        st[si].nblocks = (int32_t)(total / kBlockSyms) + 1;
    }
}

__global__ __launch_bounds__(256) void zs_fast_stitch_kernel(const StreamDesc *sd, const uint2 *work, const uint32_t *run_syms,
                                                             const FastRunOut *outs, uint32_t *syms, int32_t *blk_end,
                                                             int32_t *blk_top) {
    __shared__ long long part[256];
    const uint2 w = work[blockIdx.x];
    const StreamDesc s = sd[w.x];
    const int64_t run = (int64_t)s.run_off + w.y;
    const FastRunOut o = outs[run];
    const uint32_t *src = run_syms + run * kFastRunSyms + o.mark_nsyms;
    uint32_t *dst = syms + s.sym_off + o.sym_dst;
    const int64_t cnt = o.nsyms - o.mark_nsyms;
    const int tid = threadIdx.x;
    for (int64_t i = tid; i < cnt; i += 256) dst[i] = src[i];
    int64_t i_cut = (kBlockSyms - 1) - o.sym_dst % kBlockSyms, i_done = 0, pos = o.mark_pos;
    for (; i_cut < cnt; i_cut += kBlockSyms) {
        long long sum = 0;
        for (int64_t i = i_done + tid; i < i_cut; i += 256) {
            const uint32_t v = src[i];
            sum += (v >> 16) ? (long long)(v & 0xFFFF) + 3 : 1;
        }
        part[tid] = sum;
        __syncthreads();
        for (int k = 128; k > 0; k >>= 1) {
            if (tid < k) part[tid] += part[tid + k];
            __syncthreads();
        }
        const int64_t start = pos + part[0];
        __syncthreads();
        const uint32_t v = src[i_cut];
        pos = start + ((v >> 16) ? (int64_t)(v & 0xFFFF) + 3 : 1);
        if (tid == 0) {
            const int64_t g = o.sym_dst + i_cut;
            blk_end[s.blk_off + g / kBlockSyms] = (int32_t)pos;
            blk_top[s.blk_off + g / kBlockSyms] = (int32_t)start;
        }
        i_done = i_cut + 1;
    }
}

__global__ __launch_bounds__(64) void zs_fast_blocks_kernel(const StreamDesc *sd, const StreamState *st, const FastRunOut *outs,
                                                            const int32_t *blk_end, const int32_t *blk_top, BlockRec *blocks,
                                                            int nstreams) {
    const int si = blockIdx.x;
    const StreamDesc s = sd[si];
    if (s.fast_runs <= 0) return;
    const int nb = st[si].nblocks;
    const int64_t total = st[si].nsyms;
    for (int b = threadIdx.x; b < nb; b += 64) {
        BlockRec r;
        r.start = b ? blk_end[s.blk_off + b - 1] : 0;
        r.sym_start = (int64_t)b * kBlockSyms;
        if (b + 1 < nb) {
            r.stored_len = (int32_t)(blk_end[s.blk_off + b] - r.start);
            r.nsyms = kBlockSyms;
            r.can_store = r.start >= (int64_t)kWSize * refills_fired_at(blk_top[s.blk_off + b], s.kl);
            r.eof = 0;
        } else {
            r.stored_len = (int32_t)((int64_t)s.n - r.start);
            r.nsyms = (int32_t)(total - r.sym_start);
            r.can_store = r.start >= outs[s.run_off + s.fast_runs - 1].final_base;
            r.eof = 1;
        }
        blocks[s.blk_off + b] = r;
    }
}

#include "zs_fast_sweep.hip"
#include "zs_rle.hip"

__device__ int build_tree_wave(TreeWork &w, uint32_t *hk, uint32_t *pd, uint32_t *nc, CtData *tree, const TreeDesc &d, int lane) {
    int len = 0, max_code = -1;
    for (int base = 0; base < d.elems; base += 64) {
        const int n = base + lane;
        const uint32_t f = n < d.elems ? tree[n].fc : 0;
        const uint64_t nz = __ballot(f != 0);
        if (f) hk[len + 1 + __builtin_popcountll(nz & lanemask_lt())] = hk_pack(f, 0, (uint32_t)n);
        else if (n < d.elems) tree[n].dl = 0;
        if (nz) max_code = base + 63 - __builtin_clzll(nz);
        len += __builtin_popcountll(nz);
    }
    while (len < 2) {
        const int node = max_code < 2 ? ++max_code : 0;
        len++;
        if (lane == 0) {
            hk[len] = hk_pack(1, 0, (uint32_t)node);
            tree[node].fc = 1;
            w.opt_len--;
            if (d.which != 2) w.static_len -= desc_static_len(d, node);
        }
    }
    __threadfence_block();
    if (lane == 0) {
        w.heap_max = kHeapSize;
        int hl = len;
        for (int n = hl / 2; n >= 1; n--) pqdownheap_packed(hk, hl, n);
        int node = d.elems;
        do {
            const uint32_t n = hk[1];
            hk[1] = hk[hl--];
            pqdownheap_packed(hk, hl, 1);
            const uint32_t m = hk[1];
            w.heap[--w.heap_max] = (uint16_t)(n & 1023u);
            w.heap[--w.heap_max] = (uint16_t)(m & 1023u);
            const uint32_t f = (n >> 16) + (m >> 16), dn = (n >> 10) & 63u, dm = (m >> 10) & 63u;
            tree[node].fc = (uint16_t)f;
            tree[n & 1023u].dl = tree[m & 1023u].dl = (uint16_t)node;
            hk[1] = hk_pack(f, (dn >= dm ? dn : dm) + 1, (uint32_t)node);
            node++;
            pqdownheap_packed(hk, hl, 1);
        } while (hl >= 2);
        w.heap[--w.heap_max] = (uint16_t)(hk[1] & 1023u);
        w.heap_len = hl;
    }
    __threadfence_block();
    const int hmax = w.heap_max, root = w.heap[hmax];
    for (int h = hmax + lane; h < kHeapSize; h += 64) {
        const int n = w.heap[h];
        pd[n] = h == hmax ? ((uint32_t)n << 8) : (((uint32_t)tree[n].dl << 8) | 1u);
    }
    __threadfence_block();
    for (int r = 0; r < 6; r++) {
        for (int h = hmax + lane; h < kHeapSize; h += 64) {
            const int n = w.heap[h];
            const uint32_t v = pd[n], pv = pd[v >> 8];
            pd[n] = (pv & ~0xFFu) | ((v & 0xFFu) + (pv & 0xFFu));
        }
        __threadfence_block();
    }
    bool over = false;
    for (int h = hmax + lane; h < kHeapSize; h += 64) over |= (int)(pd[w.heap[h]] & 0xFFu) > d.max_length;
    (void)root;
    if (__ballot(over)) {
        if (lane == 0) gen_bitlen(w, tree, max_code, d);
        __threadfence_block();
    } else {
        if (lane < 16) nc[lane] = 0;
        __threadfence_block();
        int opt = 0, stat = 0;
        for (int h = hmax + lane; h < kHeapSize; h += 64) {
            const int n = w.heap[h];
            const int bits = (int)(pd[n] & 0xFFu);
            tree[n].dl = (uint16_t)bits;
            if (n <= max_code) {
                atomicAdd(&nc[bits], 1u);
                const int xbits = desc_extra(d, n), f = tree[n].fc;
                opt += f * (bits + xbits);
                if (d.which != 2) stat += f * (desc_static_len(d, n) + xbits);
            }
        }
#pragma unroll
        for (int o = 32; o >= 1; o >>= 1) opt += __shfl_xor(opt, o), stat += __shfl_xor(stat, o);
        __threadfence_block();
        if (lane <= kMaxBits) w.bl_count[lane] = (uint16_t)nc[lane];
        if (lane == 0) w.opt_len += opt, w.static_len += stat;
        __threadfence_block();
    }
    if (lane == 0) {
        unsigned code = 0;
        nc[0] = 0;
        for (int bits = 1; bits <= kMaxBits; bits++) {
            code = (code + w.bl_count[bits - 1]) << 1;
            nc[bits] = code;
        }
    }
    __threadfence_block();
    for (int base = 0; base <= max_code; base += 64) {
        const int n = base + lane;
        const int l = n <= max_code ? (int)tree[n].dl : 0;
        if (l) {
            const uint32_t code = atomicAdd(&nc[l], 1u);
            tree[n].fc = (uint16_t)(__brev(code) >> (32 - l));
        }
    }
    __threadfence_block();
    return max_code;
}
__device__ int build_block_trees_wave(TreeWork &w, uint32_t *hk, uint32_t *pd, uint32_t *nc, int stored_len, bool can_store,
                                      int strategy, int lane) {
    if (lane == 0) {
        w.opt_len = w.static_len = 0;
        for (int i = 0; i < kBlCodes; i++) w.bltree[i].fc = 0;
    }
    __threadfence_block();
    const TreeDesc ld = {0, kLCodes, kMaxBits, kLiterals + 1};
    const TreeDesc dd = {1, kDCodes, kMaxBits, 0};
    const TreeDesc bd = {2, kBlCodes, kMaxBlBits, 0};
    const int lmax = build_tree_wave(w, hk, pd, nc, w.ltree, ld, lane);
    const int dmax = build_tree_wave(w, hk, pd, nc, w.dtree, dd, lane);
    if (lane == 0) {
        w.l_max_code = lmax, w.d_max_code = dmax;
        scan_tree(w, w.ltree, lmax);
        scan_tree(w, w.dtree, dmax);
    }
    __threadfence_block();
    build_tree_wave(w, hk, pd, nc, w.bltree, bd, lane);
    int type = 2;
    if (lane == 0) {
        int mb;
        for (mb = kBlCodes - 1; mb >= 3; mb--)
            if (w.bltree[bl_order(mb)].dl != 0) break;
        w.max_blindex = mb;
        w.opt_len += 3 * (mb + 1) + 5 + 5 + 4;
        int opt_lenb = (w.opt_len + 3 + 7) >> 3;
        const int static_lenb = (w.static_len + 3 + 7) >> 3;
        if (static_lenb <= opt_lenb) opt_lenb = static_lenb;
        if (stored_len + 4 <= opt_lenb && can_store) type = 0;
        else if (strategy == kFixed || static_lenb == opt_lenb) type = 1;
    }
    return type;
}

constexpr uint32_t kNoWork = 0xFFFFFFFFu;
__global__ __launch_bounds__(1024) void zs_live_scan_kernel(const StreamState *st, int n, int32_t *live_pre) {
    __shared__ int32_t wsum[16];
    __shared__ int32_t carry;
    const int tid = threadIdx.x, lane = tid & 63, wave = tid >> 6;
    if (tid == 0) carry = 0;
    __syncthreads();
    for (int base = 0; base < n; base += 1024) {
        const int i = base + tid;
        const int32_t v = i < n && !st[i].deferred ? st[i].nblocks : 0;
        int32_t inc = v;
#pragma unroll
        for (int off = 1; off < 64; off <<= 1) {
            const int32_t o = __shfl_up(inc, off);
            if (lane >= off) inc += o;
        }
        if (lane == 63) wsum[wave] = inc;
        __syncthreads();
        int32_t before = carry;
        for (int k = 0; k < wave; k++) before += wsum[k];
        if (i < n) live_pre[i] = before + inc - v;
        __syncthreads();
        if (tid == 1023) carry = before + inc;
        __syncthreads();
    }
    if (tid == 0) live_pre[n] = carry;
}
__global__ __launch_bounds__(256) void zs_live_fill_kernel(const int32_t *live_pre, int n, uint32_t n_items, uint2 *work) {
    const uint32_t g = blockIdx.x * 256 + threadIdx.x;
    if (g >= n_items) return;
    if ((int32_t)g >= live_pre[n]) {
        work[g] = make_uint2(kNoWork, 0);
        return;
    }
    int lo = 0, hi = n - 1;
    while (lo < hi) {
        const int mid = (lo + hi + 1) >> 1;
        if (live_pre[mid] <= (int32_t)g) lo = mid;
        else hi = mid - 1;
    }
    work[g] = make_uint2((uint32_t)lo, g - (uint32_t)live_pre[lo]);
}

__global__ __launch_bounds__(256) void zs_trees_kernel(const StreamDesc *sd, const StreamState *st, const uint2 *work,
                                                       const uint32_t *syms, const BlockRec *blocks, TreeWork *trees,
                                                       BlockInfo *info, int strategy, int level, int phase) {
    __shared__ TreeWork tw;
    __shared__ uint32_t hl[kLCodes], hd[kDCodes];
    __shared__ uint32_t hk[kHeapSize + 8];
    __shared__ uint32_t pd[kHeapSize + 1], nc[16];
    uint2 w = work[blockIdx.x];
    if (w.x == kNoWork || st[w.x].deferred) return;
    const StreamDesc s = sd[w.x];
    const int b = (int)w.y;
    const int nb_body = s.fast_runs > 0 ? 0 : (int)(st[w.x].body_syms / kBlockSyms);
    if (phase == 0 ? b >= nb_body : ((phase == 1 && b < nb_body) || b >= st[w.x].nblocks)) return;
    const BlockRec r = blocks[s.blk_off + b];
    if (level == 0 && r.nsyms == 0 && s.plan_nblk > 0) {
        if (threadIdx.x == 0) {
            BlockInfo bi;
            bi.type = r.can_store ? 0 : 1;
            bi.bits = r.can_store ? 0 : 10;
            bi.bit_start = 0;
            info[s.blk_off + b] = bi;
        }
        return;
    }
    for (int i = threadIdx.x; i < kLCodes; i += blockDim.x) hl[i] = 0;
    for (int i = threadIdx.x; i < kDCodes; i += blockDim.x) hd[i] = 0;
    __syncthreads();
    const uint32_t *sy = syms + s.sym_off + r.sym_start;
    for (int i = threadIdx.x; i < r.nsyms; i += blockDim.x) {
        uint32_t v = sy[i];
        int dist = (int)(v >> 16), lc = (int)(v & 0xFFFF);
        if (dist == 0) atomicAdd(&hl[lc], 1u);
        else {
            atomicAdd(&hl[length_code(lc) + kLiterals + 1], 1u);
            atomicAdd(&hd[dist_code(dist - 1)], 1u);
        }
    }
    __syncthreads();
    for (int i = threadIdx.x; i < kHeapSize; i += blockDim.x) {
        tw.ltree[i].fc = i < kLCodes ? (uint16_t)hl[i] : 0;
        tw.ltree[i].dl = 0;
    }
    for (int i = threadIdx.x; i < 2 * kDCodes + 1; i += blockDim.x) {
        tw.dtree[i].fc = i < kDCodes ? (uint16_t)hd[i] : 0;
        tw.dtree[i].dl = 0;
    }
    for (int i = threadIdx.x; i < 2 * kBlCodes + 1; i += blockDim.x) tw.bltree[i].fc = 0, tw.bltree[i].dl = 0;
    __syncthreads();
    if (threadIdx.x == 0) tw.ltree[kEndBlock].fc = 1;
    __syncthreads();
    if (threadIdx.x < 64) {
        int type = build_block_trees_wave(tw, hk, pd, nc, r.stored_len, r.can_store != 0, strategy, (int)threadIdx.x);
        if (threadIdx.x == 0) {
        if (level == 0) type = r.can_store ? 0 : 1;
        BlockInfo bi;
        bi.type = type;
        bi.bits = type == 1 ? 3 + tw.static_len : type == 2 ? 3 + tw.opt_len : 0;
        bi.bit_start = 0;
        info[s.blk_off + b] = bi;
        }
    }
    __syncthreads();
    uint32_t *dst = (uint32_t *)&trees[s.blk_off + b];
    const uint32_t *src = (const uint32_t *)&tw;
    for (int i = threadIdx.x; i < (int)(sizeof(TreeWork) / 4); i += blockDim.x) dst[i] = src[i];
}

__device__ __forceinline__ void or_bits(uint8_t *out, int64_t pos, uint64_t v, int nbits) {
    if (nbits == 0) return;
    uint32_t *w = (uint32_t *)((uintptr_t)(out + (pos >> 3)) & ~(uintptr_t)3);
    int sh = (int)(pos - ((int64_t)((uint8_t *)w - out) << 3));
    uint64_t lo = v << sh;
    uint32_t w0 = (uint32_t)lo, w1 = (uint32_t)(lo >> 32);
    uint32_t w2 = sh ? (uint32_t)(v >> (64 - sh)) : 0;
    if (w0) atomicOr(w, w0);
    if (w1) atomicOr(w + 1, w1);
    if (w2) atomicOr(w + 2, w2);
}
struct OrBitsAt {
    uint8_t *out;
    int64_t cap;
    int64_t bit_base;
    __device__ void operator()(int64_t pos, uint32_t v, int nbits) const {
        pos -= bit_base;
        if ((pos >> 3) + 12 <= cap) or_bits(out, pos, v, nbits);
    }
};
__global__ __launch_bounds__(256) void zs_offsets_kernel(const StreamDesc *sd, StreamState *st, const BlockRec *blocks,
                                                         BlockInfo *info, const TreeWork *trees, const uint32_t *adler_pieces,
                                                         int level, int nstreams) {
    __shared__ int32_t sh_type[1024], sh_bits[1024], sh_len[1024], sh_eof[1024];
    __shared__ int64_t sh_start[1024];
    __shared__ uint32_t ad_v[256];
    __shared__ uint64_t ad_len[256];
    __shared__ int64_t sh_pos, sh_wsum[4];
    __shared__ int sh_bad;
    FlushAcct fa;
    int fa_w = 0;
    const bool flushing = sd[blockIdx.x].wr_flush != nullptr;
    const int si = blockIdx.x;
    if (st[si].deferred) return;
    const StreamDesc s = sd[si];
    StreamState &ss = st[si];
    const int nb = ss.nblocks;
    LitPersist *ps = s.persist;
    const int64_t start_bits = s.cont_bits ? ps->fa.bits : 16;
    const int64_t bit_base = s.cont_bits ? (start_bits & ~7LL) : 0;
    if (threadIdx.x == 0) sh_pos = start_bits, sh_bad = 0;
    const OrBitsAt fa_put{s.out, s.out_cap, bit_base};
    if (flushing) {
        if (s.cont_bits) fa = ps->fa;
        else fa_init(fa, s.out_chunk, level, s.raw != 0);
        if (!s.mid_write) fa_enter(fa);
    }
    if (threadIdx.x == 0 && s.cont_bits && s.out_cap > 0) s.out[0] = (uint8_t)s.carry_byte;
    __syncthreads();
    for (int b0 = 0; b0 < nb; b0 += 1024) {
        int cnt = nb - b0 < 1024 ? nb - b0 : 1024;
        for (int i = threadIdx.x; i < cnt; i += 256) {
            const BlockInfo bi = info[s.blk_off + b0 + i];
            const BlockRec r = blocks[s.blk_off + b0 + i];
            sh_type[i] = bi.type, sh_bits[i] = bi.bits, sh_len[i] = r.stored_len, sh_eof[i] = r.eof;
        }
        __syncthreads();
        int irregular = 0;
        for (int i = threadIdx.x; i < cnt; i += 256) irregular |= (sh_type[i] == 0) || (sh_eof[i] && i != cnt - 1);
        irregular = __syncthreads_or(irregular | (int)flushing);
        if (!irregular) {
            const int lane = threadIdx.x & 63, wave = threadIdx.x >> 6;
            int64_t b4[4], mine = 0;
            for (int k = 0; k < 4; k++) {
                const int i = threadIdx.x * 4 + k;
                b4[k] = i < cnt ? sh_bits[i] : 0;
                mine += b4[k];
            }
            int64_t inc = mine;
            for (int o = 1; o < 64; o <<= 1) {
                const int64_t x = __shfl_up(inc, o);
                if (lane >= o) inc += x;
            }
            if (lane == 63) sh_wsum[wave] = inc;
            __syncthreads();
            int64_t before = sh_pos;
            for (int k = 0; k < wave; k++) before += sh_wsum[k];
            int64_t pos = before + inc - mine;
            for (int k = 0; k < 4; k++) {
                const int i = threadIdx.x * 4 + k;
                if (i < cnt) sh_start[i] = pos;
                pos += b4[k];
            }
            __syncthreads();
            if (threadIdx.x == 255) {
                int64_t end = pos;
                if (sh_eof[cnt - 1] & 1) end = (end + 7) & ~7LL;
                sh_pos = end;
            }
        } else if (threadIdx.x == 0) {
            int64_t pos = sh_pos;
            for (int i = 0; i < cnt; i++) {
                if (flushing)
                    while (fa_w + 1 < s.n_wr && s.wr_blk[fa_w + 1] <= b0 + i) fa_w++, fa_enter(fa);
                sh_start[i] = pos;
                if (sh_type[i] == 0) {
                    if (sh_len[i] + 5 > (level == 0 ? 32768 : 65536)) sh_bad = 1;
                    pos += 3;
                    pos = (pos + 7) & ~7LL;
                    pos += 32 + 8LL * sh_len[i];
                } else {
                    pos += sh_bits[i];
                }
                if (sh_eof[i] & 1) pos = (pos + 7) & ~7LL;
                if (flushing) {
                    fa.bits = pos;
                    fa.last_eob_len = sh_type[i] == 0 ? 8 : sh_type[i] == 1 ? 7 : trees[s.blk_off + b0 + i].ltree[kEndBlock].dl;
                    const int f = sh_eof[i] >> 1;
                    if (f) fa_end_of_write(fa, f, fa_put);
                    else fa_after_block(fa);
                    pos = fa.bits;
                }
            }
            sh_pos = pos;
        }
        __syncthreads();
        for (int i = threadIdx.x; i < cnt; i += 256) info[s.blk_off + b0 + i].bit_start = sh_start[i] - bit_base;
        __syncthreads();
    }
    uint32_t acc = 1;
    uint64_t acc_len = 0;
    {
        const int per = (s.n_adler + 255) / 256;
        for (int k = 0; k < per; k++) {
            int i = threadIdx.x * per + k;
            if (i >= s.n_adler) break;
            int64_t len = (int64_t)s.n - (int64_t)i * kAdlerPiece;
            if (len > kAdlerPiece) len = kAdlerPiece;
            acc = adler_combine(acc, adler_pieces[s.adler_off + i], (uint64_t)len);
            acc_len += (uint64_t)len;
        }
        ad_v[threadIdx.x] = acc, ad_len[threadIdx.x] = acc_len;
    }
    __syncthreads();
    for (int off = 1; off < 256; off <<= 1) {
        if ((threadIdx.x & (2 * off - 1)) == 0) {
            ad_v[threadIdx.x] = adler_combine(ad_v[threadIdx.x], ad_v[threadIdx.x + off], ad_len[threadIdx.x + off]);
            ad_len[threadIdx.x] += ad_len[threadIdx.x + off];
        }
        __syncthreads();
    }
    if (threadIdx.x != 0) return;
    const uint32_t ad = ps ? s.adler_stream : ad_v[0];
    const int64_t pos = sh_pos;
    ss.adler = ad;
    ss.end_bits = pos;
    if (ps && !s.final_run) {
        if (flushing) fa.bits = pos, ps->fa = fa, ps->fa_valid = 1;
        const int64_t bytes = (pos - bit_base) >> 3;
        ss.out_len = bytes;
        ss.status = sh_bad ? -2 : (bytes + 8 > s.out_cap ? -5 : 0);
        return;
    }
    int64_t total = (pos - bit_base) / 8 + 4;
    ss.out_len = total;
    if (sh_bad) {
        ss.status = -2;
        return;
    }
    if (total > s.out_cap) {
        ss.status = -5;
        return;
    }
    ss.status = 0;
    if (!s.cont_bits) {
        unsigned hdr = zlib_header(level);
        s.out[0] = (uint8_t)(hdr >> 8);
        s.out[1] = (uint8_t)hdr;
    }
    uint8_t *t = s.out + (pos - bit_base) / 8;
    t[0] = (uint8_t)(ad >> 24), t[1] = (uint8_t)(ad >> 16), t[2] = (uint8_t)(ad >> 8), t[3] = (uint8_t)ad;
}

struct OrPut {
    uint8_t *out;
    int64_t pos;
    __device__ void operator()(unsigned value, int nbits) {
        or_bits(out, pos, value, nbits);
        pos += nbits;
    }
};
struct LdsTree {
    const uint32_t *t;
    struct E {
        uint16_t fc, dl;
    };
    __device__ E operator[](int i) const {
        uint32_t v = t[i];
        return {(uint16_t)v, (uint16_t)(v >> 16)};
    }
};
constexpr int kEbTile = 2048;
constexpr int kEbWords = kEbTile * 48 / 32 + 256;
struct LdsBitPut {
    uint32_t *w;
    uint32_t pos;
    __device__ void put64(uint64_t v, int nbits) {
        if (nbits == 0) return;
        const uint32_t k = pos >> 5, sh = pos & 31;
        const uint64_t lo = v << sh;
        const uint32_t w0 = (uint32_t)lo, w1 = (uint32_t)(lo >> 32), w2 = sh ? (uint32_t)(v >> (64 - sh)) : 0;
        if (w0) atomicOr(&w[k], w0);
        if (w1) atomicOr(&w[k + 1], w1);
        if (w2) atomicOr(&w[k + 2], w2);
        pos += (uint32_t)nbits;
    }
    __device__ void operator()(unsigned value, int nbits) { put64(value, nbits); }
};
__global__ __launch_bounds__(256) void zs_emit_bits_kernel(const StreamDesc *sd, const StreamState *st, const uint2 *work,
                                                           const uint32_t *syms, const BlockRec *blocks, const TreeWork *trees,
                                                           const BlockInfo *info) {
    __shared__ uint32_t lt[kLCodes], dt[kDCodes];
    __shared__ uint32_t obuf[kEbWords];
    __shared__ uint32_t wsum[4];
    __shared__ uint32_t sh_bits;
    uint2 w = work[blockIdx.x];
    if (w.x == kNoWork || st[w.x].deferred) return;
    const StreamDesc s = sd[w.x];
    const int b = (int)w.y;
    if (b >= st[w.x].nblocks || st[w.x].status != 0) return;
    const BlockRec r = blocks[s.blk_off + b];
    const BlockInfo bi = info[s.blk_off + b];
    uint8_t *out = s.out;
    const int tid = threadIdx.x, lane = lane_id(), wave = tid >> 6;
    if (bi.type == 0) {
        int64_t pos = bi.bit_start;
        if (tid == 0) or_bits(out, pos, (uint64_t)(r.eof & 1), 3);
        int64_t byte = (pos + 3 + 7) >> 3;
        if (tid == 0) {
            unsigned len = (unsigned)r.stored_len;
            out[byte] = (uint8_t)len, out[byte + 1] = (uint8_t)(len >> 8);
            out[byte + 2] = (uint8_t)~len, out[byte + 3] = (uint8_t)(~len >> 8);
        }
        const gcbytes src = as_global(s.in) + (r.start - s.abs_off);
        const gbytes_w dst = as_global(out) + byte + 4;
        typedef u32x4 __attribute__((aligned(1))) u32x4u;
        const int nvec = r.stored_len >> 4;
        for (int i = tid; i < nvec; i += 256)
            *(__attribute__((address_space(1))) u32x4u *)(dst + 16 * i) = *(const __attribute__((address_space(1))) u32x4u *)(src + 16 * i);
        for (int i = (nvec << 4) + tid; i < r.stored_len; i += 256) dst[i] = src[i];
        return;
    }
    const TreeWork &tw = trees[s.blk_off + b];
    if (bi.type == 2) {
        for (int i = tid; i < kLCodes; i += 256) lt[i] = (uint32_t)tw.ltree[i].fc | ((uint32_t)tw.ltree[i].dl << 16);
        if (tid < kDCodes) dt[tid] = (uint32_t)tw.dtree[tid].fc | ((uint32_t)tw.dtree[tid].dl << 16);
    } else {
        for (int i = tid; i < kLCodes; i += 256) lt[i] = static_lcode(i) | ((uint32_t)static_llen(i) << 16);
        if (tid < kDCodes) dt[tid] = bit_reverse((unsigned)tid, 5) | (5u << 16);
    }
    for (int i = tid; i < kEbWords; i += 256) obuf[i] = 0;
    __syncthreads();
    uint32_t *const W = (uint32_t *)((uintptr_t)out & ~(uintptr_t)3);
    int64_t cur = bi.bit_start + (int64_t)(((uintptr_t)out & 3) << 3);
    if (tid == 0) {
        LdsBitPut put{obuf, (uint32_t)(cur & 31)};
        put((unsigned)(bi.type << 1) + (unsigned)(r.eof & 1), 3);
        if (bi.type == 2) emit_dyn_header(tw, put);
        sh_bits = put.pos - (uint32_t)(cur & 31);
    }
    __syncthreads();
    LdsTree L{lt}, D{dt};
    const uint32_t *sy = syms + s.sym_off + r.sym_start;
    const int total = r.nsyms + 1;
    bool first = true;
    uint32_t pending = sh_bits;
    auto flush = [&](uint32_t nb, bool last) {
        const uint32_t end = (uint32_t)(cur & 31) + nb;
        const uint32_t nfull = end >> 5;
        uint32_t *g = W + (cur >> 5);
        const uint32_t carry = obuf[nfull];
        __syncthreads();
        for (uint32_t k = tid; k < nfull; k += 256) {
            const uint32_t v = obuf[k];
            if (k == 0 && first) {
                if (v) atomicOr(g, v);
            } else {
                g[k] = v;
            }
            obuf[k] = 0;
        }
        if (tid == 0) {
            obuf[nfull] = 0;
            if (last) {
                if (carry) atomicOr(g + nfull, carry);
            } else {
                obuf[0] = carry;
            }
        }
        if (nfull) first = false;
        cur += nb;
        __syncthreads();
    };
    for (int t0 = 0; t0 < total; t0 += kEbTile) {
        const int i0 = t0 + tid * 8;
        uint32_t v[8];
        uint32_t mybits = 0;
#pragma unroll
        for (int k = 0; k < 8; k++) {
            const int i = i0 + k;
            v[k] = i < r.nsyms ? sy[i] : (uint32_t)kEndBlock;
            uint64_t bits;
            if (i < total) mybits += (uint32_t)encode_symbol(L, D, (int)(v[k] >> 16), (int)(v[k] & 0xFFFF), bits);
        }
        uint32_t inc = mybits;
#pragma unroll
        for (int off = 1; off < 64; off <<= 1) {
            const uint32_t o = (uint32_t)__shfl_up((int)inc, off);
            if (lane >= off) inc += o;
        }
        if (lane == 63) wsum[wave] = inc;
        __syncthreads();
        uint32_t before = 0, tile_bits = 0;
#pragma unroll
        for (int k = 0; k < 4; k++) {
            const uint32_t x = wsum[k];
            if (k < wave) before += x;
            tile_bits += x;
        }
        LdsBitPut put{obuf, (uint32_t)(cur & 31) + pending + before + inc - mybits};
        uint64_t acc = 0;
        int fill = 0;
#pragma unroll
        for (int k = 0; k < 8; k++) {
            if (i0 + k < total) {
                uint64_t bits;
                const int nb = encode_symbol(L, D, (int)(v[k] >> 16), (int)(v[k] & 0xFFFF), bits);
                acc |= bits << fill;
                fill += nb;
                if (fill >= 16) {
                    int fl = fill & ~7;
                    if (fl > 56) fl = 56;
                    put.put64(acc & ((1ull << fl) - 1), fl);
                    acc >>= fl;
                    fill -= fl;
                }
            }
        }
        if (fill) put.put64(acc, fill);
        __syncthreads();
        flush(pending + tile_bits, t0 + kEbTile >= total);
        pending = 0;
    }
}

__global__ __launch_bounds__(256) void zs_adler_kernel(const StreamDesc *sd, const uint2 *work, uint32_t *pieces) {
    __shared__ uint64_t ra[256], rb[256];
    uint2 w = work[blockIdx.x];
    const StreamDesc s = sd[w.x];
    int64_t beg = (int64_t)w.y * kAdlerPiece;
    int64_t len = (int64_t)s.n - beg;
    if (len > kAdlerPiece) len = kAdlerPiece;
    const gcbytes p = as_global(s.in) + beg;
    int64_t o = (int64_t)threadIdx.x * 256;
    int64_t lt = len - o;
    if (lt > 256) lt = 256;
    if (lt < 0) lt = 0;
    uint64_t a = 0, bsum = 0;
    if (lt == 256 && (((uintptr_t)(p + o)) & 15) == 0) {
        const gcu32x4 v = (gcu32x4)(p + o);
#pragma unroll 4
        for (int g = 0; g < 16; g++) {
            const u32x4 q = v[g];
            const uint32_t w[4] = {q[0], q[1], q[2], q[3]};
            uint32_t ga = 0, gb = 0;
#pragma unroll
            for (int k = 0; k < 4; k++) {
                const uint32_t b0 = w[k] & 0xFF, b1 = (w[k] >> 8) & 0xFF, b2 = (w[k] >> 16) & 0xFF, b3 = w[k] >> 24;
                ga += b0 + b1 + b2 + b3;
                gb += (4 * k) * b0 + (4 * k + 1) * b1 + (4 * k + 2) * b2 + (4 * k + 3) * b3;
            }
            a += ga;
            bsum += (uint64_t)(256 - 16 * g) * ga - gb;
        }
    } else {
        for (int j = 0; j < lt; j++) {
            uint64_t d = p[o + j];
            a += d;
            bsum += (uint64_t)(lt - j) * d;
        }
    }
    uint64_t tailw = (uint64_t)(len - o - lt);
    ra[threadIdx.x] = a;
    rb[threadIdx.x] = lt > 0 ? bsum + tailw * a : 0;
    __syncthreads();
    for (int off = 128; off > 0; off >>= 1) {
        if (threadIdx.x < off) ra[threadIdx.x] += ra[threadIdx.x + off], rb[threadIdx.x] += rb[threadIdx.x + off];
        __syncthreads();
    }
    if (threadIdx.x == 0) {
        uint64_t s1 = (1 + ra[0]) % kAdlerBase;
        uint64_t s2 = ((uint64_t)len + rb[0]) % kAdlerBase;
        pieces[s.adler_off + w.y] = (uint32_t)((s2 << 16) | s1);
    }
}

__global__ __launch_bounds__(256) void zs_adler_finish_kernel(const StreamDesc *sd, const uint32_t *pieces, const uint8_t *const *trailer,
                                                              uint2 *res) {
    __shared__ uint32_t ad_v[256];
    __shared__ uint64_t ad_len[256];
    const StreamDesc s = sd[blockIdx.x];
    uint32_t acc = 1;
    uint64_t acc_len = 0;
    const int per = (s.n_adler + 255) / 256;
    for (int k = 0; k < per; k++) {
        const int i = threadIdx.x * per + k;
        if (i >= s.n_adler) break;
        int64_t len = (int64_t)s.n - (int64_t)i * kAdlerPiece;
        if (len > kAdlerPiece) len = kAdlerPiece;
        acc = adler_combine(acc, pieces[s.adler_off + i], (uint64_t)len);
        acc_len += (uint64_t)len;
    }
    ad_v[threadIdx.x] = acc, ad_len[threadIdx.x] = acc_len;
    __syncthreads();
    for (int off = 1; off < 256; off <<= 1) {
        if ((threadIdx.x & (2 * off - 1)) == 0) {
            ad_v[threadIdx.x] = adler_combine(ad_v[threadIdx.x], ad_v[threadIdx.x + off], ad_len[threadIdx.x + off]);
            ad_len[threadIdx.x] += ad_len[threadIdx.x + off];
        }
        __syncthreads();
    }
    if (threadIdx.x != 0) return;
    uint32_t ok = 1;
    if (trailer && trailer[blockIdx.x]) {
        const uint8_t *t = trailer[blockIdx.x];
        const uint32_t want = ((uint32_t)t[0] << 24) | ((uint32_t)t[1] << 16) | ((uint32_t)t[2] << 8) | t[3];
        ok = want == ad_v[0];
    }
    res[blockIdx.x] = make_uint2(ad_v[0], ok);
}

__device__ __forceinline__ int png_paeth(int a, int b, int c) {
    const int p = a + b - c, pa = abs(p - a), pb = abs(p - b), pc = abs(p - c);
    return (pa <= pb && pa <= pc) ? a : (pb <= pc ? b : c);
}
__device__ __forceinline__ uint8_t png_apply(int f, int x, int a, int b, int c) {
    switch (f) {
    case 1: return (uint8_t)(x - a);
    case 2: return (uint8_t)(x - b);
    case 3: return (uint8_t)(x - ((a + b) >> 1));
    case 4: return (uint8_t)(x - png_paeth(a, b, c));
    default: return (uint8_t)x;
    }
}
__global__ __launch_bounds__(256) void zs_png_filter_kernel(const uint8_t *pix, int64_t row_bytes, int64_t height, int bpp, int filter,
                                                            uint8_t *out) {
    __shared__ uint32_t sums[5][256];
    __shared__ int chosen;
    const int64_t y = blockIdx.x;
    const gcbytes cur = as_global(pix) + y * row_bytes, up = y ? cur - row_bytes : cur;
    const bool has_up = y > 0;
    int f = filter;
    if (filter == 5) {
        uint32_t acc[5] = {0, 0, 0, 0, 0};
        for (int64_t i = threadIdx.x; i < row_bytes; i += 256) {
            const int x = cur[i], a = i >= bpp ? cur[i - bpp] : 0, b = has_up ? up[i] : 0, c = (has_up && i >= bpp) ? up[i - bpp] : 0;
#pragma unroll
            for (int k = 0; k < 5; k++) {
                const int v = (int8_t)png_apply(k, x, a, b, c);
                acc[k] += (uint32_t)(v < 0 ? -v : v);
            }
        }
        for (int k = 0; k < 5; k++) sums[k][threadIdx.x] = acc[k];
        __syncthreads();
        for (int off = 128; off > 0; off >>= 1) {
            if (threadIdx.x < off)
                for (int k = 0; k < 5; k++) sums[k][threadIdx.x] += sums[k][threadIdx.x + off];
            __syncthreads();
        }
        if (threadIdx.x == 0) {
            int best = 0;
            for (int k = 1; k < 5; k++)
                if (sums[k][0] < sums[best][0]) best = k;
            chosen = best;
        }
        __syncthreads();
        f = chosen;
    }
    uint8_t *o = out + y * (row_bytes + 1);
    if (threadIdx.x == 0) o[0] = (uint8_t)f;
    for (int64_t i = threadIdx.x; i < row_bytes; i += 256) {
        const int x = cur[i], a = i >= bpp ? cur[i - bpp] : 0, b = has_up ? up[i] : 0, c = (has_up && i >= bpp) ? up[i - bpp] : 0;
        o[1 + i] = png_apply(f, x, a, b, c);
    }
}

struct PngFiltImg {
    const uint8_t *pix;
    uint8_t *out;
    int64_t row_bytes;
    int32_t bpp, filter;
};
constexpr int kPngStageRow = 16384;
constexpr int kPngStageLds = kPngStageRow + 48;

__device__ __forceinline__ int png_stage_row(uint8_t *lds, const uint8_t *g, int nbytes, int tid) {
// ... 91 lines not shown
```

Before: 15180 MB/s.

## Split emit-bits per block into tiles and build lit/dist trees on separate waves

The trees kernel now builds the literal/length tree and the distance tree concurrently on two waves, using a side work struct, vectorises the symbol histogram loads, and writes per-tile bit counts. The emit kernel launches a 2D grid. One part writes the block header, and the other parts each encode a tile of symbols at an offset computed from the precomputed tile bit counts, so tiles no longer run serially within a block. This adds extra work items and atomics at tile boundaries, plus the cost of producing tile_bits in the trees kernel.

```diff
diff --git a/zlibstream_amd/csrc/zs_core.h b/zlibstream_amd/csrc/zs_core.h
--- a/zlibstream_amd/csrc/zs_core.h
+++ b/zlibstream_amd/csrc/zs_core.h
@@ -593,6 +593,7 @@
 };
 
 struct TreeWork {
+    static constexpr int kHeap = kHeapSize;
     CtData ltree[kHeapSize];
     CtData dtree[2 * kDCodes + 1];
     CtData bltree[2 * kBlCodes + 1];
@@ -615,11 +616,12 @@
 }
 ZS_HD int desc_static_len(const TreeDesc &d, int n) { return d.which == 0 ? static_llen(n) : 5; }
 
-ZS_HD_NOINLINE inline void gen_bitlen(TreeWork &w, CtData *tree, int max_code, const TreeDesc &d) {
+template <class W>
+ZS_HD_NOINLINE inline void gen_bitlen(W &w, CtData *tree, int max_code, const TreeDesc &d) {
     int h, n, m, bits, overflow = 0;
     for (bits = 0; bits <= kMaxBits; bits++) w.bl_count[bits] = 0;
     tree[w.heap[w.heap_max]].dl = 0;
-    for (h = w.heap_max + 1; h < kHeapSize; h++) {
+    for (h = w.heap_max + 1; h < W::kHeap; h++) {
         n = w.heap[h];
         bits = tree[tree[n].dl].dl + 1;
         if (bits > d.max_length) {
@@ -738,7 +740,8 @@
     return max_code;
 }
 
-ZS_HD_NOINLINE inline void scan_tree(TreeWork &w, CtData *tree, int max_code) {
+template <class W>
+ZS_HD_NOINLINE inline void scan_tree(W &w, CtData *tree, int max_code) {
     int prevlen = -1, curlen, nextlen = tree[0].dl, count = 0, max_count = 7, min_count = 4;
     if (nextlen == 0) max_count = 138, min_count = 3;
     tree[max_code + 1].dl = 0xFFFF;
diff --git a/zlibstream_amd/csrc/zs_engine.hip b/zlibstream_amd/csrc/zs_engine.hip
--- a/zlibstream_amd/csrc/zs_engine.hip
+++ b/zlibstream_amd/csrc/zs_engine.hip
@@ -62,7 +62,7 @@
     hipEvent_t ev[kStCount + 1] = {};
     double stage_ms[kStCount] = {};
     uint32_t *crc_tab = nullptr;
-    DevBuf sd, st, work, wpre, geo, link, mm, maps, chunk_far, segmap, supmap, seg_entry, seg_symbase, seg_stale, entry, symbase, stale, syms, blk_end, blk_top, blocks, trees, info, pieces, scratch,
+    DevBuf sd, st, work, wpre, geo, link, mm, maps, chunk_far, segmap, supmap, seg_entry, seg_symbase, seg_stale, entry, symbase, stale, syms, blk_end, blk_top, blocks, trees, info, tile_bits, pieces, scratch,
         stage_in, stage_out, wr, inf_desc, inf_state, par_ps, par_st, par_work, par_cbits, par_ccnt, par_surv, par_scnt, par_cands, par_tabs, par_toktabs, par_toks, par_ctoks, par_tokstat, par_tails, par_retry, par_fxtab, par_blocks, par_cells,
         par_windows, par_fail, run_syms, run_bits, run_scratch, run_outs, run_fail, adl_tr, adl_res, plan_blk, ins_bits, mm_bak, cut_pos, cut_bkt, win_groups, win_sg, win_maps, win_entries, persist_bak, resume_flag, rle_tiles, own_in, fr_chunks, fr_meta, fr_planes, fr_prov, fr_base, fr_counters, spec_rec, spec_flags, spec_syms, png_img, png_seg, png_ctr, png_fimg, png_scratch, png_a7img, png_inflated, png_passes, crc_desc, crc_res, png_zs, png_gather, png_ximg, png_raw;
     uint32_t *crc32_tab = nullptr;
@@ -510,9 +510,10 @@
         !ensure(c, c->seg_entry, 2 * (size_t)(pl.n_segs + 2)) || !ensure(c, c->seg_symbase, 4 * (size_t)(pl.n_segs + 2)) ||
         !ensure(c, c->seg_stale, (size_t)pl.n_segs + 64) || !ensure(c, c->entry, 2 * (size_t)(pl.n_chunks + 2)) ||
         !ensure(c, c->symbase, 4 * (size_t)(pl.n_chunks + 2)) || !ensure(c, c->stale, (size_t)pl.n_chunks + 64) ||
-        !ensure(c, c->syms, 4 * (size_t)pl.n_syms + 64) || !ensure(c, c->blk_end, 4 * (size_t)pl.n_blocks + 64) ||
+        !ensure(c, c->syms, 4 * (size_t)pl.n_syms + kSymsSlack) || !ensure(c, c->blk_end, 4 * (size_t)pl.n_blocks + 64) ||
         !ensure(c, c->blk_top, 4 * (size_t)pl.n_blocks + 64) || !ensure(c, c->blocks, sizeof(BlockRec) * (size_t)pl.n_blocks) ||
         !ensure(c, c->trees, sizeof(TreeWork) * (size_t)pl.n_blocks) || !ensure(c, c->info, sizeof(BlockInfo) * (size_t)pl.n_blocks) ||
+        !ensure(c, c->tile_bits, 4 * (size_t)kEbTiles * (size_t)pl.n_blocks + 64) ||
         !ensure(c, c->pieces, 4 * (size_t)pl.n_pieces + 64) || !ensure(c, c->scratch, (size_t)kScratchBytes * (size_t)n) ||
         !ensure(c, c->cut_pos, 8 * (size_t)pl.n_cuts + 64) || !ensure(c, c->cut_bkt, 8 * (size_t)pl.n_cuts + 64) ||
         (pl.n_spec && (!ensure(c, c->spec_rec, 8 * (size_t)pl.n_spec + 64) || !ensure(c, c->spec_flags, 4 * (size_t)n + 64) ||
@@ -1029,14 +1030,23 @@
                            (uint32_t)pl.w_blocks.size(), dev<uint2>(c->work) + o_blocks);
     }
     hipLaunchKernelGGL(zs_trees_kernel, dim3((unsigned)pl.w_blocks.size()), dim3(trees_threads), 0, stream, d_sd, d_st, d_work + o_blocks,
-                       dev<uint32_t>(c->syms), dev<BlockRec>(c->blocks), dev<TreeWork>(c->trees), dev<BlockInfo>(c->info), strategy, level, 2);
+                       dev<uint32_t>(c->syms), dev<BlockRec>(c->blocks), dev<TreeWork>(c->trees), dev<BlockInfo>(c->info), dev<int32_t>(c->tile_bits), strategy, level);
     mark(11);
     ZS_HIP(c, hipStreamWaitEvent(stream, c->ev_pre, 0));
     hipLaunchKernelGGL(zs_offsets_kernel, dim3((unsigned)n), dim3(256), 0, stream, d_sd, d_st, dev<BlockRec>(c->blocks),
                        dev<BlockInfo>(c->info), dev<TreeWork>(c->trees), dev<uint32_t>(c->pieces), level, n);
     mark(12);
-    hipLaunchKernelGGL(zs_emit_bits_kernel, dim3((unsigned)pl.w_blocks.size()), dim3(256), 0, stream, d_sd, d_st, d_work + o_blocks,
-                       dev<uint32_t>(c->syms), dev<BlockRec>(c->blocks), dev<TreeWork>(c->trees), dev<BlockInfo>(c->info));
+    int eb_tiles = kEbTiles;
+    if (level != 0) {
+        int64_t longest = 0;
+        for (int i = 0; i < n; i++) longest = std::max(longest, in_len[i]);
+        eb_tiles = (int)std::min<int64_t>(kEbTiles, (longest + 1) / kEbTile + 1);
+    }
+    static const char *const eb_env = getenv("ZS_EB_TILES");
+    if (eb_env) eb_tiles = std::max(1, std::min(kEbTiles, atoi(eb_env)));
+    hipLaunchKernelGGL(zs_emit_bits_kernel, dim3((unsigned)pl.w_blocks.size(), (unsigned)(1 + eb_tiles)), dim3(256), 0, stream, d_sd, d_st,
+                       d_work + o_blocks, dev<uint32_t>(c->syms), dev<BlockRec>(c->blocks), dev<TreeWork>(c->trees), dev<BlockInfo>(c->info),
+                       dev<int32_t>(c->tile_bits));
     mark(13);
     ZS_HIP(c, hipGetLastError());
     StreamState *hst = (StreamState *)c->pinned;
@@ -1177,7 +1187,7 @@
 int batch_prefix_that_fits(zs_ctx *c, int n, const int64_t *in_len, const int64_t *out_cap, int lo, int per_byte) {
     size_t free_b = 0, total_b = 0;
     if (hipMemGetInfo(&free_b, &total_b) != hipSuccess) return n;
-    const DevBuf *held[] = {&c->link, &c->mm, &c->maps, &c->segmap, &c->supmap, &c->syms, &c->trees, &c->blocks, &c->info, &c->stage_in, &c->stage_out,
+    const DevBuf *held[] = {&c->link, &c->mm, &c->maps, &c->segmap, &c->supmap, &c->syms, &c->trees, &c->blocks, &c->info, &c->tile_bits, &c->stage_in, &c->stage_out,
                             &c->scratch, &c->ins_bits, &c->mm_bak};
     size_t have = 0;
     for (const DevBuf *b : held) have += b->cap;
@@ -1289,7 +1299,7 @@
     if (!c) return;
     (void)hipSetDevice(c->device);
     DevBuf *bufs[] = {&c->sd, &c->st, &c->work, &c->wpre, &c->geo, &c->link, &c->mm, &c->maps, &c->chunk_far, &c->segmap, &c->supmap, &c->seg_entry, &c->seg_symbase, &c->seg_stale, &c->entry, &c->symbase, &c->stale, &c->syms,
-                      &c->blk_end, &c->blk_top, &c->blocks, &c->trees, &c->info, &c->pieces, &c->scratch, &c->stage_in, &c->stage_out, &c->wr, &c->inf_desc, &c->inf_state, &c->par_ps, &c->par_st, &c->par_work, &c->par_cbits, &c->par_ccnt, &c->par_surv, &c->par_scnt,
+                      &c->blk_end, &c->blk_top, &c->blocks, &c->trees, &c->info, &c->tile_bits, &c->pieces, &c->scratch, &c->stage_in, &c->stage_out, &c->wr, &c->inf_desc, &c->inf_state, &c->par_ps, &c->par_st, &c->par_work, &c->par_cbits, &c->par_ccnt, &c->par_surv, &c->par_scnt,
                       &c->par_cands, &c->par_tabs, &c->par_toktabs, &c->par_toks, &c->par_ctoks, &c->par_tokstat, &c->par_tails, &c->par_retry, &c->par_fxtab, &c->par_blocks, &c->par_cells, &c->par_windows, &c->par_fail, &c->run_syms, &c->run_bits,
                       &c->run_scratch, &c->run_outs, &c->run_fail, &c->adl_tr, &c->adl_res, &c->plan_blk, &c->ins_bits, &c->mm_bak, &c->cut_pos, &c->cut_bkt, &c->win_groups, &c->win_sg, &c->win_maps, &c->win_entries, &c->persist_bak, &c->resume_flag, &c->rle_tiles, &c->own_in, &c->fr_chunks, &c->fr_meta, &c->fr_planes, &c->fr_prov, &c->fr_base, &c->fr_counters, &c->spec_rec, &c->spec_flags, &c->spec_syms, &c->png_img, &c->png_seg, &c->png_ctr, &c->png_fimg, &c->png_scratch, &c->png_a7img, &c->png_inflated, &c->png_passes, &c->crc_desc, &c->crc_res, &c->png_zs, &c->png_gather, &c->png_ximg, &c->png_raw};
     for (DevBuf *b : bufs)
diff --git a/zlibstream_amd/csrc/zs_kernels.hip b/zlibstream_amd/csrc/zs_kernels.hip
--- a/zlibstream_amd/csrc/zs_kernels.hip
+++ b/zlibstream_amd/csrc/zs_kernels.hip
@@ -2563,7 +2563,16 @@
 #include "zs_fast_sweep.hip"
 #include "zs_rle.hip"
 
-__device__ int build_tree_wave(TreeWork &w, uint32_t *hk, uint32_t *pd, uint32_t *nc, CtData *tree, const TreeDesc &d, int lane) {
+struct SideTree {
+    static constexpr int kHeap = 2 * kDCodes + 1;
+    uint16_t heap[kHeap];
+    uint16_t bl_count[kMaxBits + 1];
+    CtData bltree[kBlCodes];
+    int heap_len, heap_max;
+    int opt_len, static_len;
+};
+template <class W>
+__device__ int build_tree_wave(W &w, uint32_t *hk, uint32_t *pd, uint32_t *nc, CtData *tree, const TreeDesc &d, int lane) {
     int len = 0, max_code = -1;
     for (int base = 0; base < d.elems; base += 64) {
         const int n = base + lane;
@@ -2586,7 +2595,7 @@
     }
     __threadfence_block();
     if (lane == 0) {
-        w.heap_max = kHeapSize;
+        w.heap_max = W::kHeap;
         int hl = len;
         for (int n = hl / 2; n >= 1; n--) pqdownheap_packed(hk, hl, n);
         int node = d.elems;
@@ -2609,13 +2618,13 @@
     }
     __threadfence_block();
     const int hmax = w.heap_max, root = w.heap[hmax];
-    for (int h = hmax + lane; h < kHeapSize; h += 64) {
+    for (int h = hmax + lane; h < W::kHeap; h += 64) {
         const int n = w.heap[h];
         pd[n] = h == hmax ? ((uint32_t)n << 8) : (((uint32_t)tree[n].dl << 8) | 1u);
     }
     __threadfence_block();
     for (int r = 0; r < 6; r++) {
-        for (int h = hmax + lane; h < kHeapSize; h += 64) {
+        for (int h = hmax + lane; h < W::kHeap; h += 64) {
             const int n = w.heap[h];
             const uint32_t v = pd[n], pv = pd[v >> 8];
             pd[n] = (pv & ~0xFFu) | ((v & 0xFFu) + (pv & 0xFFu));
@@ -2623,7 +2632,7 @@
         __threadfence_block();
     }
     bool over = false;
-    for (int h = hmax + lane; h < kHeapSize; h += 64) over |= (int)(pd[w.heap[h]] & 0xFFu) > d.max_length;
+    for (int h = hmax + lane; h < W::kHeap; h += 64) over |= (int)(pd[w.heap[h]] & 0xFFu) > d.max_length;
     (void)root;
     if (__ballot(over)) {
         if (lane == 0) gen_bitlen(w, tree, max_code, d);
@@ -2632,7 +2641,7 @@
         if (lane < 16) nc[lane] = 0;
         __threadfence_block();
         int opt = 0, stat = 0;
-        for (int h = hmax + lane; h < kHeapSize; h += 64) {
+        for (int h = hmax + lane; h < W::kHeap; h += 64) {
             const int n = w.heap[h];
             const int bits = (int)(pd[n] & 0xFFu);
             tree[n].dl = (uint16_t)bits;
@@ -2670,24 +2679,30 @@
     __threadfence_block();
     return max_code;
 }
-__device__ int build_block_trees_wave(TreeWork &w, uint32_t *hk, uint32_t *pd, uint32_t *nc, int stored_len, bool can_store,
-                                      int strategy, int lane) {
-    if (lane == 0) {
-        w.opt_len = w.static_len = 0;
-        for (int i = 0; i < kBlCodes; i++) w.bltree[i].fc = 0;
-    }
-    __threadfence_block();
+__device__ void build_ld_tree_wave(TreeWork &w, SideTree &sw, uint32_t *hk, uint32_t *pd, uint32_t *nc, uint32_t *hk2, uint32_t *pd2,
+                                   uint32_t *nc2, int wave, int lane) {
     const TreeDesc ld = {0, kLCodes, kMaxBits, kLiterals + 1};
     const TreeDesc dd = {1, kDCodes, kMaxBits, 0};
+    if (wave == 0) {
+        const int lmax = build_tree_wave(w, hk, pd, nc, w.ltree, ld, lane);
+        if (lane == 0) {
+            w.l_max_code = lmax;
+            scan_tree(w, w.ltree, lmax);
+        }
+    } else {
+        const int dmax = build_tree_wave(sw, hk2, pd2, nc2, w.dtree, dd, lane);
+        if (lane == 0) {
+            w.d_max_code = dmax;
+            scan_tree(sw, w.dtree, dmax);
+        }
+    }
+}
+__device__ int build_bl_tree_wave(TreeWork &w, const SideTree &sw, uint32_t *hk, uint32_t *pd, uint32_t *nc, int stored_len,
+                                  bool can_store, int strategy, int lane) {
+    if (lane < kBlCodes) w.bltree[lane].fc += sw.bltree[lane].fc;
+    if (lane == 0) w.opt_len += sw.opt_len, w.static_len += sw.static_len;
+    __threadfence_block();
     const TreeDesc bd = {2, kBlCodes, kMaxBlBits, 0};
-    const int lmax = build_tree_wave(w, hk, pd, nc, w.ltree, ld, lane);
-    const int dmax = build_tree_wave(w, hk, pd, nc, w.dtree, dd, lane);
-    if (lane == 0) {
-        w.l_max_code = lmax, w.d_max_code = dmax;
-        scan_tree(w, w.ltree, lmax);
-        scan_tree(w, w.dtree, dmax);
-    }
-    __threadfence_block();
     build_tree_wave(w, hk, pd, nc, w.bltree, bd, lane);
     int type = 2;
     if (lane == 0) {
@@ -2706,6 +2721,11 @@
 }
 
 constexpr uint32_t kNoWork = 0xFFFFFFFFu;
+constexpr int kEbTile = 2048;
+constexpr int kEbTiles = 8;
+static_assert(kEbTile * kEbTiles >= kBlockSyms + 1, "a block's symbols and END_BLOCK fit its tiles");
+constexpr int kSymsSlack = 64;
+static_assert(kSymsSlack >= 16, "a 16-byte load that starts inside the symbols ends inside the array");
 __global__ __launch_bounds__(1024) void zs_live_scan_kernel(const StreamState *st, int n, int32_t *live_pre) {
     __shared__ int32_t wsum[16];
     __shared__ int32_t carry;
@@ -2748,19 +2768,32 @@
     work[g] = make_uint2((uint32_t)lo, g - (uint32_t)live_pre[lo]);
 }
 
+#ifdef ZS_BS_PROF
+#define BS_PF(i) { const long long now_ = wall_clock64(); pf[i] += now_ - pf_t; pf_t = now_; }
+#else
+#define BS_PF(i)
+#endif
+typedef u32x4 __attribute__((aligned(4))) u32x4a4;
+typedef u32x4 __attribute__((aligned(8))) u32x4a8;
 __global__ __launch_bounds__(256) void zs_trees_kernel(const StreamDesc *sd, const StreamState *st, const uint2 *work,
                                                        const uint32_t *syms, const BlockRec *blocks, TreeWork *trees,
-                                                       BlockInfo *info, int strategy, int level, int phase) {
-    __shared__ TreeWork tw;
+                                                       BlockInfo *info, int32_t *tile_bits, int strategy, int level) {
+    __shared__ __attribute__((aligned(16))) TreeWork tw;
+    __shared__ SideTree sw;
     __shared__ uint32_t hl[kLCodes], hd[kDCodes];
     __shared__ uint32_t hk[kHeapSize + 8];
     __shared__ uint32_t pd[kHeapSize + 1], nc[16];
+    __shared__ uint32_t hk2[SideTree::kHeap + 8], pd2[SideTree::kHeap + 1], nc2[16];
+    __shared__ uint32_t sh_tile[2 * kEbTiles];
+    __shared__ int sh_type;
+#ifdef ZS_BS_PROF
+    long long pf[8] = {0, 0, 0, 0, 0, 0, 0, 0}, pf_t = wall_clock64();
+#endif
     uint2 w = work[blockIdx.x];
     if (w.x == kNoWork || st[w.x].deferred) return;
     const StreamDesc s = sd[w.x];
     const int b = (int)w.y;
-    const int nb_body = s.fast_runs > 0 ? 0 : (int)(st[w.x].body_syms / kBlockSyms);
-    if (phase == 0 ? b >= nb_body : ((phase == 1 && b < nb_body) || b >= st[w.x].nblocks)) return;
+    if (b >= st[w.x].nblocks) return;
     const BlockRec r = blocks[s.blk_off + b];
     if (level == 0 && r.nsyms == 0 && s.plan_nblk > 0) {
         if (threadIdx.x == 0) {
@@ -2772,48 +2805,148 @@
         }
         return;
     }
-    for (int i = threadIdx.x; i < kLCodes; i += blockDim.x) hl[i] = 0;
-    for (int i = threadIdx.x; i < kDCodes; i += blockDim.x) hd[i] = 0;
-    __syncthreads();
+    const int tid = (int)threadIdx.x, nthr = (int)blockDim.x, lane = tid & 63, wave = tid >> 6;
+    for (int i = tid; i < kLCodes; i += nthr) hl[i] = 0;
+    for (int i = tid; i < kDCodes; i += nthr) hd[i] = 0;
+    if (tid < 2 * kEbTiles) sh_tile[tid] = 0;
+    __syncthreads();
+    BS_PF(0);
     const uint32_t *sy = syms + s.sym_off + r.sym_start;
-    for (int i = threadIdx.x; i < r.nsyms; i += blockDim.x) {
-        uint32_t v = sy[i];
-        int dist = (int)(v >> 16), lc = (int)(v & 0xFFFF);
+    auto tally = [&](uint32_t v) {
+        const int dist = (int)(v >> 16), lc = (int)(v & 0xFFFF);
         if (dist == 0) atomicAdd(&hl[lc], 1u);
         else {
             atomicAdd(&hl[length_code(lc) + kLiterals + 1], 1u);
             atomicAdd(&hd[dist_code(dist - 1)], 1u);
         }
-    }
-    __syncthreads();
-    for (int i = threadIdx.x; i < kHeapSize; i += blockDim.x) {
+    };
+    {
+        const int nvec = r.nsyms >> 2;
+        const __attribute__((address_space(1))) u32x4a4 *sv = (const __attribute__((address_space(1))) u32x4a4 *)(uintptr_t)sy;
+        int i = tid;
+        for (; i + 3 * nthr < nvec; i += 4 * nthr) {
+            const u32x4 q0 = sv[i], q1 = sv[i + nthr], q2 = sv[i + 2 * nthr], q3 = sv[i + 3 * nthr];
+#pragma unroll
+            for (int k = 0; k < 4; k++) tally(q0[k]);
+#pragma unroll
+            for (int k = 0; k < 4; k++) tally(q1[k]);
+#pragma unroll
+            for (int k = 0; k < 4; k++) tally(q2[k]);
+#pragma unroll
+            for (int k = 0; k < 4; k++) tally(q3[k]);
+        }
+        for (; i < nvec; i += nthr) {
+            const u32x4 q = sv[i];
+#pragma unroll
+            for (int k = 0; k < 4; k++) tally(q[k]);
+        }
+        for (int j = (nvec << 2) + tid; j < r.nsyms; j += nthr) tally(sy[j]);
+    }
+    __syncthreads();
+    BS_PF(1);
+    for (int i = tid; i < kHeapSize; i += nthr) {
         tw.ltree[i].fc = i < kLCodes ? (uint16_t)hl[i] : 0;
         tw.ltree[i].dl = 0;
     }
-    for (int i = threadIdx.x; i < 2 * kDCodes + 1; i += blockDim.x) {
+    for (int i = tid; i < 2 * kDCodes + 1; i += nthr) {
         tw.dtree[i].fc = i < kDCodes ? (uint16_t)hd[i] : 0;
         tw.dtree[i].dl = 0;
     }
-    for (int i = threadIdx.x; i < 2 * kBlCodes + 1; i += blockDim.x) tw.bltree[i].fc = 0, tw.bltree[i].dl = 0;
-    __syncthreads();
-    if (threadIdx.x == 0) tw.ltree[kEndBlock].fc = 1;
-    __syncthreads();
-    if (threadIdx.x < 64) {
-        int type = build_block_trees_wave(tw, hk, pd, nc, r.stored_len, r.can_store != 0, strategy, (int)threadIdx.x);
-        if (threadIdx.x == 0) {
-        if (level == 0) type = r.can_store ? 0 : 1;
-        BlockInfo bi;
-        bi.type = type;
-        bi.bits = type == 1 ? 3 + tw.static_len : type == 2 ? 3 + tw.opt_len : 0;
-        bi.bit_start = 0;
-        info[s.blk_off + b] = bi;
-        }
-    }
-    __syncthreads();
-    uint32_t *dst = (uint32_t *)&trees[s.blk_off + b];
-    const uint32_t *src = (const uint32_t *)&tw;
-    for (int i = threadIdx.x; i < (int)(sizeof(TreeWork) / 4); i += blockDim.x) dst[i] = src[i];
-}
+    for (int i = tid; i < 2 * kBlCodes + 1; i += nthr) tw.bltree[i].fc = 0, tw.bltree[i].dl = 0;
+    if (tid < kBlCodes) sw.bltree[tid].fc = 0, sw.bltree[tid].dl = 0;
+    if (tid == 0) tw.opt_len = tw.static_len = 0, sw.opt_len = sw.static_len = 0;
+    __syncthreads();
+    if (tid == 0) tw.ltree[kEndBlock].fc = 1;
+    __syncthreads();
+    BS_PF(2);
+    if (wave < 2) build_ld_tree_wave(tw, sw, hk, pd, nc, hk2, pd2, nc2, wave, lane);
+#ifdef ZS_BS_PROF
+    if (wave == 1) BS_PF(4);
+#endif
+    __syncthreads();
+    BS_PF(3);
+    const int total = r.nsyms + 1;
+    const bool tiled = total > kEbTile;
+    if (tiled) {
+        for (int i = tid; i < kLCodes; i += nthr) {
+            const uint32_t x = i > kLiterals ? (uint32_t)extra_lbits(i - kLiterals - 1) : 0;
+            hl[i] = (((uint32_t)tw.ltree[i].dl + x) & 0xFFu) | (((uint32_t)static_llen(i) + x) << 8);
+        }
+        for (int i = tid; i < kDCodes; i += nthr) {
+            const uint32_t x = (uint32_t)extra_dbits(i);
+            hd[i] = (((uint32_t)tw.dtree[i].dl + x) & 0xFFu) | ((5u + x) << 8);
+        }
+        __syncthreads();
+    }
+    if (wave == 0) {
+        int type = build_bl_tree_wave(tw, sw, hk, pd, nc, r.stored_len, r.can_store != 0, strategy, lane);
+        if (lane == 0) {
+            if (level == 0) type = r.can_store ? 0 : 1;
+            BlockInfo bi;
+            bi.type = type;
+            bi.bits = type == 1 ? 3 + tw.static_len : type == 2 ? 3 + tw.opt_len : 0;
+            bi.bit_start = 0;
+            info[s.blk_off + b] = bi;
+            sh_type = type;
+        }
+    } else if (tiled) {
+        const int wk = tid - 64, nwk = nthr - 64;
+        const __attribute__((address_space(1))) u32x4a4 *sv = (const __attribute__((address_space(1))) u32x4a4 *)(uintptr_t)sy;
+        uint32_t dyn[kEbTiles], stat[kEbTiles];
+#pragma unroll
+        for (int t = 0; t < kEbTiles; t++) {
+            dyn[t] = stat[t] = 0;
+            if (t * kEbTile < total) {
+                const int nv = ((total < (t + 1) * kEbTile ? total : (t + 1) * kEbTile) - t * kEbTile + 3) >> 2;
+#pragma unroll 4
+                for (int j = wk; j < nv; j += nwk) {
+                    const u32x4 q = sv[t * (kEbTile / 4) + j];
+#pragma unroll
+                    for (int k = 0; k < 4; k++) {
+                        const int i = t * kEbTile + 4 * j + k;
+                        const uint32_t v = q[k];
+                        const int dist = (int)(v >> 16), lc = (int)(v & 0xFFFF);
+                        uint32_t e = 0;
+                        if (i < r.nsyms) e = dist == 0 ? hl[lc] : hl[length_code(lc) + kLiterals + 1] + hd[dist_code(dist - 1)];
+                        else if (i == r.nsyms) e = hl[kEndBlock];
+                        dyn[t] += e & 0xFFu;
+                        stat[t] += e >> 8;
+                    }
+                }
+            }
+        }
+#pragma unroll
+        for (int t = 0; t < kEbTiles; t++) {
+            if (t * kEbTile < total) {
+                uint32_t a = dyn[t], c = stat[t];
+#pragma unroll
+                for (int o = 32; o >= 1; o >>= 1) a += __shfl_xor(a, o), c += __shfl_xor(c, o);
+                if (lane == 0) atomicAdd(&sh_tile[t], a), atomicAdd(&sh_tile[kEbTiles + t], c);
+            }
+        }
+    }
+    __syncthreads();
+    BS_PF(5);
+    {
+        __attribute__((address_space(1))) u32x4a8 *dv = (__attribute__((address_space(1))) u32x4a8 *)(uintptr_t)&trees[s.blk_off + b];
+        const u32x4 *src4 = (const u32x4 *)&tw;
+        constexpr int nw = (int)(sizeof(TreeWork) / 4);
+        for (int i = tid; i < nw / 4; i += nthr) dv[i] = src4[i];
+        uint32_t *dst = (uint32_t *)&trees[s.blk_off + b];
+        const uint32_t *src = (const uint32_t *)&tw;
+        if (tid < (nw & 3)) dst[(nw & ~3) + tid] = src[(nw & ~3) + tid];
+    }
+    BS_PF(6);
+    const int type = sh_type;
+    if (tiled && type != 0 && tid < kEbTiles) tile_bits[(int64_t)(s.blk_off + b) * kEbTiles + tid] = (int32_t)sh_tile[(type == 2 ? 0 : kEbTiles) + tid];
+#ifdef ZS_BS_PROF
+    BS_PF(7);
+    if (lane == 0 && wave < 2 && (blockIdx.x & 255) == 7)
+        printf("BSPROF K7 block %d wave %d nsyms %d type %d ticks(100MHz): zero=%lld histogram=%lld fill=%lld ltree+scan/wait=%lld dtree+scan=%lld bltree+type (tile bits beside it)=%lld copy-out=%lld tile bits out=%lld\n",
+               (int)blockIdx.x, wave, r.nsyms, type, pf[0], pf[1], pf[2], pf[3], pf[4], pf[5], pf[6], pf[7]);
+#endif
+}
+#undef BS_PF
 
 __device__ __forceinline__ void or_bits(uint8_t *out, int64_t pos, uint64_t v, int nbits) {
     if (nbits == 0) return;
@@ -3006,7 +3139,6 @@
         return {(uint16_t)v, (uint16_t)(v >> 16)};
     }
 };
-constexpr int kEbTile = 2048;
 constexpr int kEbWords = kEbTile * 48 / 32 + 256;
 struct LdsBitPut {
     uint32_t *w;
@@ -3023,13 +3155,21 @@
     }
     __device__ void operator()(unsigned value, int nbits) { put64(value, nbits); }
 };
+#ifdef ZS_BS_PROF
+#define BS_PF(i) { const long long now_ = wall_clock64(); pf[i] += now_ - pf_t; pf_t = now_; }
+#else
+#define BS_PF(i)
+#endif
 __global__ __launch_bounds__(256) void zs_emit_bits_kernel(const StreamDesc *sd, const StreamState *st, const uint2 *work,
                                                            const uint32_t *syms, const BlockRec *blocks, const TreeWork *trees,
-                                                           const BlockInfo *info) {
+                                                           const BlockInfo *info, const int32_t *tile_bits) {
     __shared__ uint32_t lt[kLCodes], dt[kDCodes];
     __shared__ uint32_t obuf[kEbWords];
     __shared__ uint32_t wsum[4];
     __shared__ uint32_t sh_bits;
+#ifdef ZS_BS_PROF
+    long long pf[4] = {0, 0, 0, 0}, pf_t = wall_clock64();
+#endif
     uint2 w = work[blockIdx.x];
     if (w.x == kNoWork || st[w.x].deferred) return;
     const StreamDesc s = sd[w.x];
@@ -3039,11 +3179,12 @@
     const BlockInfo bi = info[s.blk_off + b];
     uint8_t *out = s.out;
     const int tid = threadIdx.x, lane = lane_id(), wave = tid >> 6;
+    const int part = (int)blockIdx.y, ntl = (int)gridDim.y - 1;
     if (bi.type == 0) {
         int64_t pos = bi.bit_start;
-        if (tid == 0) or_bits(out, pos, (uint64_t)(r.eof & 1), 3);
         int64_t byte = (pos + 3 + 7) >> 3;
-        if (tid == 0) {
+        if (part == 0 && tid == 0) {
+            or_bits(out, pos, (uint64_t)(r.eof & 1), 3);
             unsigned len = (unsigned)r.stored_len;
             out[byte] = (uint8_t)len, out[byte + 1] = (uint8_t)(len >> 8);
             out[byte + 2] = (uint8_t)~len, out[byte + 3] = (uint8_t)(~len >> 8);
@@ -3052,12 +3193,57 @@
         const gbytes_w dst = as_global(out) + byte + 4;
         typedef u32x4 __attribute__((aligned(1))) u32x4u;
         const int nvec = r.stored_len >> 4;
-        for (int i = tid; i < nvec; i += 256)
+        for (int i = part * 256 + tid; i < nvec; i += 256 * (int)gridDim.y)
             *(__attribute__((address_space(1))) u32x4u *)(dst + 16 * i) = *(const __attribute__((address_space(1))) u32x4u *)(src + 16 * i);
-        for (int i = (nvec << 4) + tid; i < r.stored_len; i += 256) dst[i] = src[i];
+        if (part == 0)
+            for (int i = (nvec << 4) + tid; i < r.stored_len; i += 256) dst[i] = src[i];
         return;
     }
+    uint32_t *const W = (uint32_t *)((uintptr_t)out & ~(uintptr_t)3);
+    const int64_t cur0 = bi.bit_start + (int64_t)(((uintptr_t)out & 3) << 3);
+    auto flush = [&](int64_t cur, uint32_t nb) {
+        const uint32_t nw = ((uint32_t)(cur & 31) + nb + 31) >> 5;
+        uint32_t *g = W + (cur >> 5);
+        for (uint32_t k = tid; k < nw; k += 256) {
+            const uint32_t v = obuf[k];
+            if (k == 0 || k == nw - 1) {
+                if (v) atomicOr(g + k, v);
+            } else {
+                g[k] = v;
+            }
+            obuf[k] = 0;
+        }
+        __syncthreads();
+    };
     const TreeWork &tw = trees[s.blk_off + b];
+    if (part == 0) {
+        if (bi.type == 1) {
+            if (tid == 0) or_bits(out, bi.bit_start, 2u + (unsigned)(r.eof & 1), 3);
+            return;
+        }
+        constexpr int kHdrWords = 160, kTwWords = (int)(sizeof(TreeWork) / 4);
+        static_assert(kHdrWords + kTwWords <= kEbWords && sizeof(TreeWork) % 4 == 0, "the header and a TreeWork fit obuf");
+        for (int i = tid; i < kHdrWords; i += 256) obuf[i] = 0;
+        for (int i = tid; i < kTwWords; i += 256) obuf[kHdrWords + i] = ((const uint32_t *)&tw)[i];
+        __syncthreads();
+        if (tid == 0) {
+            LdsBitPut put{obuf, (uint32_t)(cur0 & 31)};
+            put(4u + (unsigned)(r.eof & 1), 3);
+            emit_dyn_header(*(const TreeWork *)(obuf + kHdrWords), put);
+            sh_bits = put.pos - (uint32_t)(cur0 & 31);
+        }
+        __syncthreads();
+        BS_PF(1);
+        flush(cur0, sh_bits);
+#ifdef ZS_BS_PROF
+        BS_PF(3);
+        if (tid == 0 && (blockIdx.x & 255) == 7) printf("BSPROF K9 block %d header ticks(100MHz): header=%lld flush=%lld\n", (int)blockIdx.x, pf[1], pf[3]);
+#endif
+        return;
+    }
+    const int total = r.nsyms + 1;
+    const int ntiles = (total + kEbTile - 1) / kEbTile;
+    if (part - 1 >= ntiles) return;
     if (bi.type == 2) {
         for (int i = tid; i < kLCodes; i += 256) lt[i] = (uint32_t)tw.ltree[i].fc | ((uint32_t)tw.ltree[i].dl << 16);
         if (tid < kDCodes) dt[tid] = (uint32_t)tw.dtree[tid].fc | ((uint32_t)tw.dtree[tid].dl << 16);
@@ -3067,49 +3253,14 @@
     }
     for (int i = tid; i < kEbWords; i += 256) obuf[i] = 0;
     __syncthreads();
-    uint32_t *const W = (uint32_t *)((uintptr_t)out & ~(uintptr_t)3);
-    int64_t cur = bi.bit_start + (int64_t)(((uintptr_t)out & 3) << 3);
-    if (tid == 0) {
-        LdsBitPut put{obuf, (uint32_t)(cur & 31)};
-        put((unsigned)(bi.type << 1) + (unsigned)(r.eof & 1), 3);
-        if (bi.type == 2) emit_dyn_header(tw, put);
-        sh_bits = put.pos - (uint32_t)(cur & 31);
-    }
-    __syncthreads();
+    BS_PF(0);
     LdsTree L{lt}, D{dt};
     const uint32_t *sy = syms + s.sym_off + r.sym_start;
-    const int total = r.nsyms + 1;
-    bool first = true;
-    uint32_t pending = sh_bits;
-    auto flush = [&](uint32_t nb, bool last) {
-        const uint32_t end = (uint32_t)(cur & 31) + nb;
-        const uint32_t nfull = end >> 5;
-        uint32_t *g = W + (cur >> 5);
-        const uint32_t carry = obuf[nfull];
-        __syncthreads();
-        for (uint32_t k = tid; k < nfull; k += 256) {
-            const uint32_t v = obuf[k];
-            if (k == 0 && first) {
-                if (v) atomicOr(g, v);
-            } else {
-                g[k] = v;
-            }
-            obuf[k] = 0;
-        }
-        if (tid == 0) {
-            obuf[nfull] = 0;
-            if (last) {
-                if (carry) atomicOr(g + nfull, carry);
-            } else {
-                obuf[0] = carry;
-            }
-        }
-        if (nfull) first = false;
-        cur += nb;
-        __syncthreads();
-    };
-    for (int t0 = 0; t0 < total; t0 += kEbTile) {
-        const int i0 = t0 + tid * 8;
+    const int32_t *tb = tile_bits + (int64_t)(s.blk_off + b) * kEbTiles;
+    for (int t = part - 1; t < ntiles; t += ntl) {
+        uint32_t later = 0;
+        for (int u = t + 1; u < ntiles; u++) later += (uint32_t)tb[u];
+        const int i0 = t * kEbTile + tid * 8;
         uint32_t v[8];
         uint32_t mybits = 0;
 #pragma unroll
@@ -3127,14 +3278,15 @@
         }
         if (lane == 63) wsum[wave] = inc;
         __syncthreads();
-        uint32_t before = 0, tile_bits = 0;
+        uint32_t before = 0, mine = 0;
 #pragma unroll
         for (int k = 0; k < 4; k++) {
             const uint32_t x = wsum[k];
             if (k < wave) before += x;
-            tile_bits += x;
-        }
-        LdsBitPut put{obuf, (uint32_t)(cur & 31) + pending + before + inc - mybits};
+            mine += x;
+        }
+        const int64_t cur = cur0 + (int64_t)((uint32_t)bi.bits - later - mine);
+        LdsBitPut put{obuf, (uint32_t)(cur & 31) + before + inc - mybits};
         uint64_t acc = 0;
         int fill = 0;
 #pragma unroll
@@ -3155,9 +3307,14 @@
         }
         if (fill) put.put64(acc, fill);
         __syncthreads();
-        flush(pending + tile_bits, t0 + kEbTile >= total);
-        pending = 0;
-    }
+        BS_PF(2);
+        flush(cur, mine);
+        BS_PF(3);
+    }
+#ifdef ZS_BS_PROF
+    if (tid == 0 && (blockIdx.x & 255) == 7)
+        printf("BSPROF K9 block %d part %d ticks(100MHz): tables=%lld tile=%lld flush=%lld\n", (int)blockIdx.x, part, pf[0], pf[2], pf[3]);
+#endif
 }
 
 __global__ __launch_bounds__(256) void zs_adler_kernel(const StreamDesc *sd, const uint2 *work, uint32_t *pieces) {
```

Result: faster. 15420 MB/s (median of 6 runs) (+1.6%).
